# retinal-information-processing-lab/gaussian_processes

Measured on AMD Instinct MI355X. Metric: GP fits/sec (kernel+chol+solve+grad loglik) at N=8192 d=256, higher is better.
Workload: dtype f64; 1 GPU; N=8192 d=256 single cell f64, one M-step closure evaluation with 6 gradients (BASELINE configs[2], headline); N=8192, d=256, parallelism=independent units over 1 GPU(s), one process per GPU, no data-path collective

## Files before the change

gaussian_processes_amd/_lib.py:

```python
from __future__ import annotations

import ctypes
import os

from .build import lib_path

vp, i32, i64, f64 = ctypes.c_void_p, ctypes.c_int, ctypes.c_int64, ctypes.c_double
pd = ctypes.POINTER(ctypes.c_double)



class DevGemmArgs(ctypes.Structure):
    _fields_ = ([(n, vp) for n in ("A", "B", "C")] + [(n, i64) for n in ("lda", "ldb", "ldc", "sA", "sB", "sC")] +
                [("alpha", f64), ("beta", f64)] +
                [(n, vp) for n in ("sk_ws", "aux", "sumsq", "Ap", "Bp", "Cp", "auxp", "sumsqp")] +
                [(n, ctypes.c_int32) for n in ("M", "N", "K", "a_kmajor", "b_kmajor", "out_lower", "a_tri", "b_tri", "batch",
                                               "split_k", "tile", "walk", "epi", "nptr", "k_slabs")])


class DevGemmRoute(ctypes.Structure):
    _fields_ = [(n, ctypes.c_int32) for n in ("rc", "tile", "sk_first", "xcd", "stages", "half_occ", "edge", "epi",
                                              "sumsq_entries", "blocks", "pair", "slabs")]


_SIGS = {
    "gpfit_version": (i32, []),
    "gpfit_last_error": (ctypes.c_char_p, []),
    "gpfit_dgemm": (i32, [vp, i32, i32, i32, i32, i32, f64, vp, i64, vp, i64, f64, vp, i64, i32, i32, i32]),
    "gpfit_dgemm_ex": (i32, [vp, i32, i32, i32, i32, i32, f64, vp, i64, vp, i64, f64, vp, i64, i32, i32, i32, i32, i32]),
    "gpfit_ctx_create": (i32, [i32, i64, i64, i64, ctypes.POINTER(vp)]),
    "gpfit_ctx_destroy": (None, [vp]),
    "gpfit_check_limits": (i32, [pd, pd, pd]),
    "gpfit_localker_mask": (i32, [pd, i32, i32, vp, ctypes.POINTER(i64)]),
    "gpfit_localker": (i32, [vp, vp, pd, i32, i32, vp, i64, vp, vp]),
    "gpfit_acosker": (i32, [vp, vp, f64, vp, i64, i64, vp, i64, i64, i64, vp, i64, vp, vp, i64, vp]),
    "gpfit_acosker_pullback": (i32, [vp, vp, f64, vp, i64, i64, vp, i64, i64, i64, vp, i64, vp, i64, vp, vp, i64, pd]),
    "gpfit_acosker_diag": (i32, [vp, vp, f64, vp, i64, i64, i64, vp, i64, vp, vp, vp]),
    "gpfit_fit_eval": (i32, [vp, vp, pd, pd, pd, i32, i32, vp, i64, i64, vp, vp, vp, i64, f64, f64, i32, pd,
                             vp, vp, vp]),
    "gpfit_potrf": (i32, [vp, vp, vp, i64, i64, vp, i64, vp, i64, pd, ctypes.POINTER(i32)]),
    "gpfit_potrf_append": (i32, [vp, vp, vp, i64, vp, i64, i64, vp, pd, ctypes.POINTER(i32)]),
    "gpfit_estep": (i32, [vp, vp, vp, i64, i64, vp, vp, vp, f64, vp, vp, i64]),
    "gpfit_estep_projected": (i32, [vp, vp, vp, i64, vp, i64, vp, i64, i64, i64, vp, vp, vp, f64, vp, vp, i64, vp, vp,
                                    vp]),
    "gpfit_fparam_eval": (i32, [vp, vp, vp, vp, vp, i64, f64, i32, f64, vp, pd]),
    "gpfit_fparam_lbfgs": (i32, [vp, vp, vp, vp, vp, i64, f64, i32, f64, i32, i32, f64, f64, f64, vp, pd]),
    "gpfit_estep_chain": (i32, [vp, vp, vp, i64, vp, i64, vp, i64, i64, i64, vp, vp, vp, vp, vp, i64, vp, vp, f64, i32, f64,
                                i32, i32, i32, f64, f64, f64, pd]),
    "gpfit_estep_chain_full": (i32, [vp, vp, vp, i64, i64, vp, vp, vp, vp, vp, i64, vp, vp, f64, i32, f64, i32, i32, i32, f64,
                                     f64, f64, pd]),
    "gpfit_estep_chain_batch": (i32, [vp, i32, vp, vp, vp, vp, vp, vp, vp, i64, vp, vp, vp, vp, vp, vp, vp, vp, vp, pd, i32, pd,
                                      i32, i32, i32, f64, f64, f64, pd]),
    "gpfit_fparam_lbfgs_host": (i32, [vp, vp, vp, i64, f64, i32, f64, i32, i32, f64, f64, f64, vp, pd]),
    "gpfit_set_profile": (i32, [vp, i32]),
    "gpfit_get_profile": (i32, [vp, pd]),
    "gpfit_get_phases": (i32, [vp, pd]),
    "gpfit_last_enqueue_ms": (f64, [vp]),
    "gpfit_fit_eval_f32": (i32, [vp, vp, pd, pd, pd, i32, i32, vp, i64, i64, vp, vp, vp, i64, f64, f64, i32, pd,
                                 vp, vp, vp]),
    "gpfit_fit_eval_finish": (i32, [vp, pd]),
    "gpfit_fit_eval_batch": (i32, [vp, i32, vp, pd, pd, pd, i32, i32, vp, i64, i64, vp, vp, vp, i64, pd, pd, i32, pd,
                                   ctypes.POINTER(i32)]),
    "gpfit_fit_eval_batch_f32": (i32, [vp, i32, vp, pd, pd, pd, i32, i32, vp, i64, i64, vp, vp, vp, i64, pd, pd, i32, pd,
                                       ctypes.POINTER(i32)]),
    "gpfit_fit_eval_projected": (i32, [vp, vp, pd, pd, pd, i32, i32, vp, i64, i64, vp, vp, i64, i64, vp, vp, i64, f64, f64, pd]),
    "gpfit_fit_eval_sparse": (i32, [vp, vp, pd, pd, pd, i32, i32, vp, i64, i64, vp, i64, i64, vp, vp, i64, i64, vp, vp, i64,
                                    f64, f64, pd]),
    "gpfit_fit_eval_sparse_batch": (i32, [vp, i32, vp, pd, pd, pd, i32, i32, vp, i64, i64, vp, i64, i64, vp, vp, vp, vp, vp,
                                          vp, vp, pd, pd, pd, ctypes.POINTER(i32)]),
    "gpfit_grad_pullback": (i32, [vp, vp, pd, i32, i32, vp, i64, i64, vp, i64, vp, pd]),
    "gpfit_nd_utility": (i32, [vp, vp, vp, i64, vp, i32, vp]),
    "gpfit_probe_mfma_f64": (i32, [vp, vp, i32, i32]),
    "gpfit_probe_stream_copy": (i32, [vp, vp, vp, i64]),
    "gpfit_dev_gemm_route": (i32, [i32, ctypes.POINTER(DevGemmArgs), ctypes.POINTER(DevGemmArgs), ctypes.POINTER(DevGemmRoute)]),
    "gpfit_dev_gemm_plan": (i64, [i32, ctypes.POINTER(DevGemmArgs), i32, ctypes.POINTER(ctypes.c_int32), i64]),
    "gpfit_dev_gemm": (i32, [vp, i32, ctypes.POINTER(DevGemmArgs), ctypes.POINTER(DevGemmArgs)]),
    "gpfit_dev_ctx_copy": (i32, [vp, ctypes.c_char_p, i64, vp, i64, i32]),
    "gpfit_dev_ctx_fill": (i32, [vp, ctypes.c_char_p, i32]),
}

_lib = None


class GpfitError(RuntimeError):
    pass


def exported_symbols():
    return sorted(_SIGS)


def load():
    global _lib
    if _lib is not None:
        return _lib
    path = lib_path()
    if not os.path.exists(path):
        raise GpfitError(
            f"{path} not found: build it with `python -m gaussian_processes_amd.build` "
            "(there is no CPU fallback for the GP fit path)")
    lib = ctypes.CDLL(path)
    for name, (res, args) in _SIGS.items():
        fn = getattr(lib, name)
        fn.restype = res
        fn.argtypes = args
    _lib = lib
    return lib


def last_error() -> str:
    return load().gpfit_last_error().decode(errors="replace")


def check(rc: int, what: str):
    if rc < 0 and rc != -2:
        raise GpfitError(f"{what} failed (rc={rc}): {last_error()}")
    return rc


def darr(values):
    return (ctypes.c_double * len(values))(*[float(v) for v in values])
```

gaussian_processes_amd/csrc/api_dev.hip:

```cpp
#include "gemm_core.h"
#include "context.h"
#include "gpfit_mi355x.h"

#include <cstring>

namespace gpfit {
namespace {

template <typename R>
int fill(const gpfit_dev_gemm_args& d, GemmArgsT<R>& g) {
  g = GemmArgsT<R>{};
  g.A = (const R*)d.A; g.B = (const R*)d.B; g.C = (R*)d.C;
  g.lda = d.lda; g.ldb = d.ldb; g.ldc = d.ldc;
  g.M = d.M; g.N = d.N; g.K = d.K;
  g.alpha = d.alpha; g.beta = d.beta;
  g.a_kmajor = d.a_kmajor; g.b_kmajor = d.b_kmajor;
  g.out_lower = d.out_lower; g.a_tri = d.a_tri; g.b_tri = d.b_tri;
  g.batch = d.batch > 0 ? d.batch : 1;
  g.sA = d.sA; g.sB = d.sB; g.sC = d.sC;
  g.split_k = d.split_k > 0 ? d.split_k : 1;
  g.k_slabs = d.k_slabs > 0 ? d.k_slabs : 0;
  g.tile = d.tile;
  g.reverse = d.walk & 15;
  g.half_occ = (d.walk >> 4) & 1;
  g.sk_ws = d.sk_ws;
  g.epi = d.epi;
  g.aux = (R*)d.aux;
  g.sumsq = d.sumsq;
  g.nptr = d.nptr;
  if (d.nptr < 0 || d.nptr > GEMM_MAXB) return d.nptr < 0 ? -3 : 0;
  for (int b = 0; b < d.nptr; ++b) {
    if (!d.Ap || !d.Bp || !d.Cp) return -3;
    g.Ap[b] = (const R*)d.Ap[b];
    g.Bp[b] = (const R*)d.Bp[b];
    g.Cp[b] = (R*)d.Cp[b];
    g.auxp[b] = d.auxp ? (R*)d.auxp[b] : nullptr;
    g.sumsqp[b] = d.sumsqp ? d.sumsqp[b] : nullptr;
  }
  return 0;
}

template <typename R>
int route(const gpfit_dev_gemm_args& d, const gpfit_dev_gemm_args* d2, gpfit_dev_gemm_route_t& o) {
  std::memset(&o, 0, sizeof(o));
  o.sk_first = -1;
  GemmArgsT<R> a, b;
  if (fill(d, a) != 0 || (d2 && fill(*d2, b) != 0)) return -3;
  GemmRoute r = d2 ? gemm_pair_shape(a, b) : gemm_route(a);
  long blocks = d2 ? r.tiles : -1;
  if (r.rc == 0 && r.sched == GEMM_STREAMK) {
    SkHostPlan plan;
    if (streamk_plan_host(a, r.sk_first, plan) != 0) r.stay_data_parallel();
    else blocks = plan.blocks;
  }
  if (r.rc == 0 && r.sched == GEMM_XCD) {
    std::vector<int> table;
    if (xcd_plan_host(a, table) != 0) return -3;
    r.gx = (int)table.size();
  }
  o.rc = r.rc; o.tile = r.tile; o.sk_first = r.sk_first; o.xcd = r.sched == GEMM_XCD; o.stages = r.stages;
  o.half_occ = r.half; o.edge = r.edge; o.epi = r.epi; o.sumsq_entries = r.sumsq_entries; o.slabs = r.slabs;
  o.pair = d2 && r.rc == 0;
  o.blocks = (int)std::min<long>(blocks >= 0 ? blocks : (long)r.gx * r.gy * r.gz, 0x7fffffffL);
  return 0;
}

template <typename R>
int64_t plan(const gpfit_dev_gemm_args& d, int kind, int32_t* out, int64_t cap) {
  GemmArgsT<R> a;
  if (fill(d, a) != 0 || a.M <= 0 || a.N <= 0) return -3;
  const GemmRoute r = gemm_route(a);
  if (r.rc != 0) return -3;
  if (kind == 1) {
    if (r.sched != GEMM_XCD) return -1;
    std::vector<int> table;
    if (xcd_plan_host(a, table) != 0) return -1;
    const int64_t need = 1 + (int64_t)table.size();
    if (need > cap || !out) return need;
    out[0] = (int32_t)table.size();
    std::memcpy(out + 1, table.data(), table.size() * sizeof(int));
    return need;
  }
  if (kind == 3) {
    if (a.k_slabs <= 0) return -1;
    const SlabPlan sp = slab_plan(a.M, a.k_slabs);
    const int64_t need = 4 + 4 * (int64_t)sp.items;
    if (need > cap || !out) return need;
    out[0] = sp.items; out[1] = sp.live; out[2] = sp.ks * SLAB_TILE; out[3] = SLAB_TILE;
    for (int e = 0; e < sp.items; ++e) {
      int ti, z;
      slab_item(sp, e, ti, z);
      int32_t* w = out + 4 + 4 * e;
      w[0] = ti; w[1] = z;
      const KRange kr = gemm_tile_k_range(a.a_tri, a.b_tri, a.K, ti * SLAB_TILE, 0, SLAB_TILE);
      w[2] = std::max(kr.beg, z * sp.ks * SLAB_TILE);
      w[3] = std::min(kr.end, (z + 1) * sp.ks * SLAB_TILE);
    }
    return need;
  }
  if (kind != 2) return -3;
  if (r.sched != GEMM_STREAMK) return -1;
  const int first = r.sk_first;
  SkHostPlan p;
  if (streamk_plan_host(a, first, p) != 0) return -1;
  const int64_t nt = (int64_t)p.tiles.size(), nfix = (int64_t)p.fix_tile.size(), nslot = (int64_t)p.fix_slot.size();
  const int64_t need = 8 + 5 * nt + nfix + (nfix + 1) + nslot;
  if (need > cap || !out) return need;
  out[0] = first; out[1] = (int32_t)nt; out[2] = p.total; out[3] = p.blocks; out[4] = p.per_block;
  out[5] = (int32_t)nfix; out[6] = (int32_t)nslot;
  out[7] = (int32_t)(SK_WS_BYTES / ((size_t)TILE * TILE * sizeof(double)));
  int32_t* w = out + 8;
  for (const SkTile& t : p.tiles) { *w++ = t.row0; *w++ = t.col0; *w++ = t.kbeg; *w++ = t.ksteps; *w++ = t.prefix; }
  std::memcpy(w, p.fix_tile.data(), nfix * sizeof(int)); w += nfix;
  std::memcpy(w, p.fix_ptr.data(), (nfix + 1) * sizeof(int)); w += nfix + 1;
  std::memcpy(w, p.fix_slot.data(), nslot * sizeof(int));
  return need;
}

template <typename R>
int run(hipStream_t s, const gpfit_dev_gemm_args& d, const gpfit_dev_gemm_args* d2) {
  GemmArgsT<R> a, b;
  if (fill(d, a) != 0 || (d2 && fill(*d2, b) != 0)) {
    set_error("gpfit_dev_gemm: a pointer batch needs its pointer arrays");
    return -3;
  }
  return d2 ? launch_gemm_pair(a, b, gemm_pair_shape(a, b), s) : launch_gemm(a, s);
}

struct CtxBuf { void* p; int64_t bytes; };
CtxBuf ctx_buffer(gpfit_ctx* c, const char* name) {
  const int64_t np = c->np_cap, dp = c->dp_cap, nn = np * np * 8;
  const struct { const char* n; double* p; int64_t bytes; } tab[] = {
      {"Abuf", c->Abuf, nn}, {"Tbuf", c->Tbuf, nn}, {"Wbuf", c->Wbuf, nn}, {"Zbuf", c->Zbuf, nn}, {"Cos", c->Cos, nn},
      {"TmpV", c->TmpV, nn}, {"Xm", c->Xm, np * dp * 8}, {"Xt2", c->Xt2, np * dp * 8}, {"Ybuf", c->Ybuf, np * dp * 8},
      {"Mmat", c->Mmat, dp * dp * 8}, {"Cmat", c->Cmat, dp * dp * 8}, {"tvec", c->tvec, 2 * np * 8}, {"bv", c->bv, np * 8},
      {"q", c->q, np * 8}, {"wl", c->wl, np * 8}, {"q2", c->q2, np * 8}, {"dq1", c->dq1, np * 8}, {"dq2", c->dq2, np * 8}};
  for (const auto& t : tab)
    if (std::strcmp(t.n, name) == 0) return {t.p, t.bytes};
  return {nullptr, 0};
}

}
}

extern "C" {

int gpfit_dev_gemm_route(int is_f32, const gpfit_dev_gemm_args* args, const gpfit_dev_gemm_args* pair_args,
                         gpfit_dev_gemm_route_t* out) {
  if (!args || !out) return -3;
  return is_f32 ? gpfit::route<float>(*args, pair_args, *out) : gpfit::route<double>(*args, pair_args, *out);
}

int64_t gpfit_dev_gemm_plan(int is_f32, const gpfit_dev_gemm_args* args, int kind, int32_t* out, int64_t cap) {
  if (!args) return -3;
  return is_f32 ? gpfit::plan<float>(*args, kind, out, cap) : gpfit::plan<double>(*args, kind, out, cap);
}

int gpfit_dev_gemm(void* stream, int is_f32, const gpfit_dev_gemm_args* args, const gpfit_dev_gemm_args* pair_args) {
  if (!args) return -3;
  return is_f32 ? gpfit::run<float>((hipStream_t)stream, *args, pair_args)
                : gpfit::run<double>((hipStream_t)stream, *args, pair_args);
}

int gpfit_dev_ctx_copy(gpfit_ctx* ctx, const char* name, int64_t offset, void* dev, int64_t bytes, int to_ctx) {
  if (!ctx || !name || !dev || offset < 0 || bytes < 0 || ctx->pend.active) return -3;
  gpfit::DeviceGuard guard(ctx->device);
  const gpfit::CtxBuf b = gpfit::ctx_buffer(ctx, name);
  if (!b.p || offset + bytes > b.bytes) return -3;
  GP_HIP(hipDeviceSynchronize());
  char* w = (char*)b.p + offset;
  GP_HIP(hipMemcpy(to_ctx ? (void*)w : dev, to_ctx ? dev : (void*)w, (size_t)bytes, hipMemcpyDeviceToDevice));
  GP_HIP(hipDeviceSynchronize());
  return 0;
}

int gpfit_dev_ctx_fill(gpfit_ctx* ctx, const char* name, int byte) {
  if (!ctx || !name || ctx->pend.active) return -3;
  gpfit::DeviceGuard guard(ctx->device);
  const gpfit::CtxBuf b = gpfit::ctx_buffer(ctx, name);
  if (!b.p) return -3;
  GP_HIP(hipDeviceSynchronize());
  GP_HIP(hipMemset(b.p, byte, (size_t)b.bytes));
  GP_HIP(hipDeviceSynchronize());
  return 0;
}

}
```

gaussian_processes_amd/csrc/chol_leaf_reg.hip:

```cpp
#include "gemm_core.h"
#include "kernels.h"

#include <cstdlib>

namespace gpfit {

#ifdef GPFIT_LEAF_STAMPS
__device__ long long g_leaf_stamps[9 * 8];
__device__ long long g_leaf_wave_end[8 * 4];
#ifdef GPFIT_LEAF_STAMPS_MIN
#define LEAF_STAMP(kb, ph) do { if (((ph) == 3 || (kb) == 8) && (threadIdx.x & 63) == 0) g_leaf_stamps[(kb) * 8 + (ph)] = (long long)__builtin_readcyclecounter(); } while (0)
#else
#define LEAF_STAMP(kb, ph) do { if ((threadIdx.x & 63) == 0) g_leaf_stamps[(kb) * 8 + (ph)] = (long long)__builtin_readcyclecounter(); } while (0)
#endif
#define LEAF_WAVE_END(kb, w) do { if ((threadIdx.x & 63) == 0) g_leaf_wave_end[(kb) * 4 + (w)] = (long long)__builtin_readcyclecounter(); } while (0)
#else
#define LEAF_STAMP(kb, ph) do { } while (0)
#define LEAF_WAVE_END(kb, w) do { } while (0)
#endif

__device__ __forceinline__ void lds_barrier() { asm volatile("s_waitcnt lgkmcnt(0)\n\ts_barrier" ::: "memory"); }
__device__ __forceinline__ void lds_fence() { asm volatile("s_waitcnt lgkmcnt(0)" ::: "memory"); }

constexpr int RL = 128;
constexpr int RPS = 18;
constexpr int RL_THREADS = 320;
constexpr int RL_TILE_THREADS = 256;

__device__ __forceinline__ double rl_readlane(double v, int src_lane) {
  const int lo = __builtin_amdgcn_readlane(__double2loint(v), src_lane);
  const int hi = __builtin_amdgcn_readlane(__double2hiint(v), src_lane);
  return __hiloint2double(hi, lo);
}
__device__ __forceinline__ float rl_readlane(float v, int src_lane) {
  return __int_as_float(__builtin_amdgcn_readlane(__float_as_int(v), src_lane));
}
template <int J, typename R> __device__ __forceinline__ R rl_rowbcast(R x) {
  return __builtin_amdgcn_update_dpp(x, x, 0x150 + J, 0xf, 0xf, false);
}

__device__ __forceinline__ void rl_rsqrt_sqrt(double p, double& rinv, double& root) {
  double y = __builtin_amdgcn_rsq(p);
  const double hp = 0.5 * p;
  y = y * fma(-hp * y, y, 1.5);
#ifdef GPFIT_LEAF_TWO_NEWTON
  y = y * fma(-hp * y, y, 1.5);
#endif
  double d = p * y;
  d = fma(fma(-d, d, p), 0.5 * y, d);
  rinv = y;
  root = d;
}
__device__ __forceinline__ void rl_rsqrt_sqrt(float p, float& rinv, float& root) {
  float y = __builtin_amdgcn_rsqf(p);
  const float hp = 0.5f * p;
  y = y * fmaf(-hp * y, y, 1.5f);
  float d = p * y;
  d = fmaf(fmaf(-d, d, p), 0.5f * y, d);
  rinv = y;
  root = d;
}

template <int J> __device__ __forceinline__ double dpp_bcast_nop(double x) {
  double r;
  asm volatile("s_nop 1\n\tv_mov_b64_dpp %0, %1 row_newbcast:%2 row_mask:0xf bank_mask:0xf" : "=v"(r) : "v"(x), "n"(J));
  return r;
}
template <int J> __device__ __forceinline__ float dpp_bcast_nop(float x) {
  float r;
  asm volatile("s_nop 1\n\tv_mov_b32_dpp %0, %1 row_newbcast:%2 row_mask:0xf bank_mask:0xf" : "=v"(r) : "v"(x), "n"(J));
  return r;
}
template <int J, bool NOP> __device__ __forceinline__ void dpp_fmac(double& acc, double a, double b) {
  if constexpr (NOP)
    asm volatile("s_nop 1\n\tv_fmac_f64_dpp %0, %1, %2 row_newbcast:%3 row_mask:0xf bank_mask:0xf" : "+v"(acc) : "v"(a), "v"(b), "n"(J));
  else
    asm volatile("v_fmac_f64_dpp %0, %1, %2 row_newbcast:%3 row_mask:0xf bank_mask:0xf" : "+v"(acc) : "v"(a), "v"(b), "n"(J));
}
template <int J, bool NOP> __device__ __forceinline__ void dpp_fmac(float& acc, float a, float b) {
  if constexpr (NOP)
    asm volatile("s_nop 1\n\tv_fmac_f32_dpp %0, %1, %2 row_newbcast:%3 row_mask:0xf bank_mask:0xf" : "+v"(acc) : "v"(a), "v"(b), "n"(J));
  else
    asm volatile("v_fmac_f32_dpp %0, %1, %2 row_newbcast:%3 row_mask:0xf bank_mask:0xf" : "+v"(acc) : "v"(a), "v"(b), "n"(J));
}

template <int J, bool NOP> __device__ __forceinline__ void dpp_fmac_self(double& x, double b) {
  if constexpr (NOP)
    asm volatile("s_nop 1\n\tv_fmac_f64_dpp %0, %0, %1 row_newbcast:%2 row_mask:0xf bank_mask:0xf" : "+v"(x) : "v"(b), "n"(J));
  else
    asm volatile("v_fmac_f64_dpp %0, %0, %1 row_newbcast:%2 row_mask:0xf bank_mask:0xf" : "+v"(x) : "v"(b), "n"(J));
}
template <int J, bool NOP> __device__ __forceinline__ void dpp_fmac_self(float& x, float b) {
  if constexpr (NOP)
    asm volatile("s_nop 1\n\tv_fmac_f32_dpp %0, %0, %1 row_newbcast:%2 row_mask:0xf bank_mask:0xf" : "+v"(x) : "v"(b), "n"(J));
  else
    asm volatile("v_fmac_f32_dpp %0, %0, %1 row_newbcast:%2 row_mask:0xf bank_mask:0xf" : "+v"(x) : "v"(b), "n"(J));
}

template <typename R, int K, int J> __device__ __forceinline__ void static_for_cols(R (&v)[16], R vk, R nvk);
template <typename R, int K, int C> __device__ __forceinline__ void static_for_inv(R (&yh)[4], R m);

template <typename R, int K>
__device__ __forceinline__ void static_for_pivots(R (&v)[16], R (&yh)[4], R& myr, int& first_bad, int lane, int base) {
  if constexpr (K < 16) {
    R p = dpp_bcast_nop<K>(v[K]);
    const bool bad = !(p > (R)0);
    first_bad = (bad && first_bad == 0) ? (base + K + 1) : first_bad;
    p = bad ? (R)1 : p;
    R rinv, dkk;
    rl_rsqrt_sqrt(p, rinv, dkk);
    myr = (lane == K) ? rinv : myr;
    const R vk = (lane == K) ? dkk : v[K] * rinv;
    v[K] = vk;
    static_for_cols<R, K, K + 1>(v, vk, -vk);
    const R m = (lane > K) ? -vk * rinv : (R)0;
    static_for_inv<R, K, 0>(yh, m);
    static_for_pivots<R, K + 1>(v, yh, myr, first_bad, lane, base);
  }
}
template <typename R, int K, int J>
__device__ __forceinline__ void static_for_cols(R (&v)[16], R vk, R nvk) {
  if constexpr (J < 16) {
    dpp_fmac<J, J == K + 1>(v[J], vk, nvk);
    static_for_cols<R, K, J + 1>(v, vk, nvk);
  }
}
template <typename R, int K, int C>
__device__ __forceinline__ void static_for_inv(R (&yh)[4], R m) {
  if constexpr (4 * C <= K) {
    dpp_fmac_self<K, C == 0>(yh[C], m);
    static_for_inv<R, K, C + 1>(yh, m);
  }
}

constexpr int RL_SLOTS = 11;
__host__ __device__ constexpr int rl_col_a(int w) { return w == 0 ? 6 : w - 1; }
__host__ __device__ constexpr int rl_col_b(int w) { return w == 0 ? 7 : 6 - w; }
__host__ __device__ constexpr int rl_nslots(int w) { return (8 - rl_col_a(w)) + (8 - rl_col_b(w)); }
__host__ __device__ constexpr int rl_slot_i(int w, int t) { return t < 8 - rl_col_a(w) ? rl_col_a(w) + t : rl_col_b(w) + (t - (8 - rl_col_a(w))); }
__host__ __device__ constexpr int rl_slot_j(int w, int t) { return t < 8 - rl_col_a(w) ? rl_col_a(w) : rl_col_b(w); }

template <typename R, int W, int C, int T0>
__device__ __forceinline__ void leaf_update_column(typename Real<R>::acc_t (&acc)[RL_SLOTS], const R* __restrict__ P,
                                                   const R (&dneg)[4], const typename Real<R>::acc_t& dvt, R* __restrict__ RawN,
                                                   R* __restrict__ Dg0, R* __restrict__ Dg1, int kb, const int (&kr)[4], int fr) {
  using Acc = typename Real<R>::acc_t;
  constexpr int NR = 8 - C;
  const int nx = kb + 1;
  R fa[2][4];
  auto row_frag = [&](int i, R (&f)[4]) {
#pragma unroll
    for (int r = 0; r < 4; ++r) f[r] = P[(16 * i + fr) * RPS + kr[r]];
  };
  if (C > kb) {
    R nfb[4];
#pragma unroll
    for (int r = 0; r < 4; ++r) nfb[r] = -P[(16 * C + fr) * RPS + kr[r]];
    row_frag(C, fa[0]);
#pragma unroll
    for (int t = 0; t < NR; ++t) {
      const int i = C + t;
      Acc& a = acc[T0 + t];
      if (t + 1 < NR) row_frag(i + 1, fa[(t + 1) & 1]);
      const R (&f)[4] = fa[t & 1];
      if (!(t == 0 && C == nx)) {
#pragma unroll
        for (int r = 0; r < 4; ++r) a = Real<R>::mfma(f[r], nfb[r], a);
      }
      if (C == nx && t > 0) {
#pragma unroll
        for (int r = 0; r < 4; ++r) RawN[(16 * i + kr[r]) * RPS + fr] = a[r];
      } else if (C == nx + 1 && t == 0) {
        R* Dg = (C & 1) ? Dg1 : Dg0;
#pragma unroll
        for (int r = 0; r < 4; ++r) Dg[kr[r] * RPS + fr] = a[r];
      }
      __builtin_amdgcn_sched_barrier(0);
    }
  } else {
    Acc xrow = acc_zero<R>();
#pragma unroll
    for (int t = 0; t < NR; ++t) {
      if (C + t == kb) {
        if (C == kb) {
          xrow = dvt;
        } else {
#pragma unroll
          for (int r = 0; r < 4; ++r) xrow = Real<R>::mfma(dneg[r], acc[T0 + t][r], xrow);
        }
        acc[T0 + t] = xrow;
      }
    }
    row_frag(C, fa[0]);
#pragma unroll
    for (int t = 0; t < NR; ++t) {
      const int i = C + t;
      Acc& a = acc[T0 + t];
      if (t + 1 < NR) row_frag(i + 1, fa[(t + 1) & 1]);
      const R (&f)[4] = fa[t & 1];
      if (i > kb) {
        if (C == kb) a = acc_zero<R>();
#pragma unroll
        for (int r = 0; r < 4; ++r) a = Real<R>::mfma(f[r], xrow[r], a);
      }
      __builtin_amdgcn_sched_barrier(0);
    }
  }
}

template <typename R, int W>
__device__ __forceinline__ void leaf_update_pass(typename Real<R>::acc_t (&acc)[RL_SLOTS], const R* __restrict__ P,
                                                 const R* __restrict__ Dv, R* __restrict__ RawN, R* __restrict__ Dg0,
                                                 R* __restrict__ Dg1, int kb, const int (&kr)[4], int fr) {
  using Acc = typename Real<R>::acc_t;
  constexpr int CA = rl_col_a(W), CB = rl_col_b(W);
  R dneg[4];
  Acc dvt;
#pragma unroll
  for (int r = 0; r < 4; ++r) {
    dneg[r] = -Dv[fr * RPS + kr[r]];
    dvt[r] = Dv[kr[r] * RPS + fr];
  }
  leaf_update_column<R, W, CA, 0>(acc, P, dneg, dvt, RawN, Dg0, Dg1, kb, kr, fr);
  leaf_update_column<R, W, CB, 8 - CA>(acc, P, dneg, dvt, RawN, Dg0, Dg1, kb, kr, fr);
}

template <typename R, int W>
__device__ __forceinline__ void leaf_load_tiles(typename Real<R>::acc_t (&acc)[RL_SLOTS], const R* __restrict__ A, int64_t lda,
                                                R* __restrict__ Raw0, R* __restrict__ Dg0, R* __restrict__ Dg1,
                                                const int (&kr)[4], int fr) {
#pragma unroll
  for (int t = 0; t < RL_SLOTS; ++t) {
    if (t >= rl_nslots(W)) { acc[t] = acc_zero<R>(); continue; }
    const int i = rl_slot_i(W, t), j = rl_slot_j(W, t);
#pragma unroll
    for (int r = 0; r < 4; ++r) acc[t][r] = A[(int64_t)(16 * i + kr[r]) * lda + 16 * j + fr];
    if (j == 0 && i > 0) {
#pragma unroll
      for (int r = 0; r < 4; ++r) Raw0[(16 * i + kr[r]) * RPS + fr] = acc[t][r];
    }
    if (i == j && j <= 1) {
      R* Dg = j ? Dg1 : Dg0;
#pragma unroll
      for (int r = 0; r < 4; ++r) Dg[kr[r] * RPS + fr] = acc[t][r];
    }
  }
}
template <typename R, int W>
__device__ __forceinline__ void leaf_store_inverse(const typename Real<R>::acc_t (&acc)[RL_SLOTS], R* __restrict__ Linv,
                                                   int64_t ldi, const int (&kr)[4], int fr) {
#pragma unroll
  for (int t = 0; t < rl_nslots(W); ++t) {
    const int i = rl_slot_i(W, t), j = rl_slot_j(W, t);
#pragma unroll
    for (int r = 0; r < 4; ++r) Linv[(int64_t)(16 * i + kr[r]) * ldi + 16 * j + fr] = acc[t][r];
  }
}

template <typename R>
__global__ __launch_bounds__(RL_THREADS, 2) void chol_leaf_reg_kernel(LeafBatchT<R> bt) {
  const R* __restrict__ A = bt.A[blockIdx.x];
  R* __restrict__ L = bt.L[blockIdx.x];
  R* __restrict__ Linv = bt.Li[blockIdx.x];
  int* __restrict__ info = bt.info[blockIdx.x];
  const int64_t lda = bt.lda, ldl = bt.ldl, ldi = bt.ldi;
  const int info_base = bt.info_base;
  using Acc = typename Real<R>::acc_t;
  using V = typename Real<R>::vec_t;
  constexpr int EPC = Real<R>::EPC;
  __shared__ __attribute__((aligned(16))) R Rawb[1][RL * RPS];
  __shared__ __attribute__((aligned(16))) R Lpb[1][RL * RPS];
  __shared__ __attribute__((aligned(16))) R Dbuf[2][16 * RPS];
  __shared__ __attribute__((aligned(16))) R Dgb[2][16 * RPS];
  __shared__ __attribute__((aligned(16))) R Sx[16 * RPS];
  __shared__ unsigned b2_arrivals;
  const int tid = threadIdx.x, lane = tid & 63;
  const int wave = __builtin_amdgcn_readfirstlane(tid >> 6);
  const int fr = lane & 15;
  int kr[4];
#pragma unroll
  for (int r = 0; r < 4; ++r) kr[r] = Real<R>::crow(lane, r);

  if (tid == 0) b2_arrivals = 0u;
  auto b2_arrive = [&]() {
    asm volatile("s_waitcnt lgkmcnt(0)" ::: "memory");
    if (lane == 0) __hip_atomic_fetch_add(&b2_arrivals, 1u, __ATOMIC_RELAXED, __HIP_MEMORY_SCOPE_WORKGROUP);
  };
  auto b2_wait = [&](unsigned target) {
    while (__hip_atomic_load(&b2_arrivals, __ATOMIC_RELAXED, __HIP_MEMORY_SCOPE_WORKGROUP) < target) { }
    asm volatile("" ::: "memory");
  };
  if (wave == 4) {
    __builtin_amdgcn_s_setprio(3);
    LEAF_STAMP(8, 0);
    auto pivot_block = [&](int nx, int lane_o) {
      const int li = lane_o & 15, lg = lane_o >> 4;
      R v[16], yh[4];
      {
        const R* row = Sx + li * RPS;
#pragma unroll
        for (int q = 0; q < 16 / EPC; ++q) {
          const V w = *reinterpret_cast<const V*>(row + EPC * q);
#pragma unroll
          for (int e = 0; e < EPC; ++e) v[EPC * q + e] = w[e];
        }
      }
#pragma unroll
      for (int c = 0; c < 4; ++c) yh[c] = (4 * c + lg == li) ? (R)1 : (R)0;
      int first_bad = 0;
      R myr = (R)0;
      LEAF_STAMP(nx, 1);
      static_for_pivots<R, 0>(v, yh, myr, first_bad, li, 16 * nx);
      LEAF_STAMP(nx, 2);
      if (lane == 0 && first_bad != 0) atomicCAS(info, 0, info_base + first_bad);
      {
        R* drow = Dbuf[nx & 1] + li * RPS + lg;
#pragma unroll
        for (int c = 0; c < 4; ++c) drow[4 * c] = yh[c] * myr;
      }
      if (lane < 16) {
        R* grow = L + (int64_t)(16 * nx + lane) * ldl + 16 * nx;
#pragma unroll
        for (int q = 0; q < 16 / EPC; ++q) {
          V lv;
#pragma unroll
          for (int e = 0; e < EPC; ++e) {
            const int j = EPC * q + e;
            lv[e] = (j <= lane) ? v[j] : (R)0;
          }
          *reinterpret_cast<V*>(grow + EPC * q) = lv;
        }
      }
      LEAF_STAMP(nx, 3);
    };
    {
      int lane_o = lane;
      asm volatile("" : "+v"(lane_o));
      if (lane < 16) {
        const R* arow = A + (int64_t)lane * lda;
        R* srow = Sx + lane * RPS;
#pragma unroll
        for (int q = 0; q < 16 / EPC; ++q) *reinterpret_cast<V*>(srow + EPC * q) = *reinterpret_cast<const V*>(arow + EPC * q);
      }
      lds_fence();
      pivot_block(0, lane_o);
    }
    lds_barrier();
#pragma unroll 1
    for (int kb = 0; kb < 8; ++kb) {
      int lane_o = lane;
      asm volatile("" : "+v"(lane_o));
      const int nx = kb + 1;
      const R* const Raw = Rawb[0];
      const R* const Dv = Dbuf[kb & 1];
      lds_barrier();
      LEAF_STAMP(kb, 4);
      if (nx < 8) {
        Acc lt = acc_zero<R>();
#pragma unroll
        for (int r = 0; r < 4; ++r) lt = Real<R>::mfma(Dv[fr * RPS + kr[r]], Raw[(16 * nx + fr) * RPS + kr[r]], lt);
        Acc sd;
#pragma unroll
        for (int r = 0; r < 4; ++r) sd[r] = Dgb[nx & 1][kr[r] * RPS + fr];
        b2_arrive();
#pragma unroll
        for (int r = 0; r < 4; ++r) sd = Real<R>::mfma(-lt[r], lt[r], sd);
#pragma unroll
        for (int r = 0; r < 4; ++r) Sx[kr[r] * RPS + fr] = sd[r];
        lds_fence();
      } else {
        b2_arrive();
      }
      LEAF_STAMP(kb, 5);
      if (nx < 8) {
        LEAF_STAMP(nx, 0);
        pivot_block(nx, lane_o);
      }
    }
    return;
  }

  Acc acc[RL_SLOTS];
  switch (wave) {
    case 0: leaf_load_tiles<R, 0>(acc, A, lda, Rawb[0], Dgb[0], Dgb[1], kr, fr); break;
    case 1: leaf_load_tiles<R, 1>(acc, A, lda, Rawb[0], Dgb[0], Dgb[1], kr, fr); break;
    case 2: leaf_load_tiles<R, 2>(acc, A, lda, Rawb[0], Dgb[0], Dgb[1], kr, fr); break;
    default: leaf_load_tiles<R, 3>(acc, A, lda, Rawb[0], Dgb[0], Dgb[1], kr, fr); break;
  }
  lds_barrier();

#pragma unroll 1
  for (int kb = 0; kb < 8; ++kb) {
    int lane_o = lane;
    asm volatile("" : "+v"(lane_o));
    const int fr = lane_o & 15;
    int kr[4];
#pragma unroll
    for (int r = 0; r < 4; ++r) kr[r] = Real<R>::crow(lane_o, r);
    const R* const Raw = Rawb[0];
    R* const P = Lpb[0];
    const R* const Dv = Dbuf[kb & 1];
    R* const RawN = Rawb[0];

    lds_barrier();
    {
      Acc s0 = acc_zero<R>(), s1 = acc_zero<R>();
      const int i0 = kb + 1 + wave, i1 = kb + 5 + wave;
      const int c0 = i0 < 8 ? i0 : 7, c1 = i1 < 8 ? i1 : 7;
      {
        R a0[4], a1[4], dd[4];
#pragma unroll
        for (int r = 0; r < 4; ++r) {
          a0[r] = Raw[(16 * c0 + fr) * RPS + kr[r]];
          a1[r] = Raw[(16 * c1 + fr) * RPS + kr[r]];
          dd[r] = Dv[fr * RPS + kr[r]];
        }
#pragma unroll
        for (int r = 0; r < 4; ++r) {
          s0 = Real<R>::mfma(a0[r], dd[r], s0);
          s1 = Real<R>::mfma(a1[r], dd[r], s1);
        }
      }
      if (i0 < 8) {
#pragma unroll
        for (int r = 0; r < 4; ++r) {
          P[(16 * i0 + kr[r]) * RPS + fr] = s0[r];
          L[(int64_t)(16 * i0 + kr[r]) * ldl + 16 * kb + fr] = s0[r];
        }
      }
      if (i1 < 8) {
#pragma unroll
        for (int r = 0; r < 4; ++r) {
          P[(16 * i1 + kr[r]) * RPS + fr] = s1[r];
          L[(int64_t)(16 * i1 + kr[r]) * ldl + 16 * kb + fr] = s1[r];
        }
      }
    }
    b2_arrive();
    b2_wait(5u * (unsigned)(kb + 1));
    switch (wave) {
      case 0: leaf_update_pass<R, 0>(acc, P, Dv, RawN, Dgb[0], Dgb[1], kb, kr, fr); break;
      case 1: leaf_update_pass<R, 1>(acc, P, Dv, RawN, Dgb[0], Dgb[1], kb, kr, fr); break;
      case 2: leaf_update_pass<R, 2>(acc, P, Dv, RawN, Dgb[0], Dgb[1], kb, kr, fr); break;
      default: leaf_update_pass<R, 3>(acc, P, Dv, RawN, Dgb[0], Dgb[1], kb, kr, fr); break;
    }
    if (wave == 0) {
      const int row = 16 * kb + (lane_o >> 2), cq = 4 * (lane_o & 3);
      V zero2;
#pragma unroll
      for (int e = 0; e < EPC; ++e) zero2[e] = (R)0;
      for (int tj = kb + 1; tj < 8; ++tj) {
        R* lrow = L + (int64_t)row * ldl + 16 * tj + cq;
        R* irow = Linv + (int64_t)row * ldi + 16 * tj + cq;
#pragma unroll
        for (int q = 0; q < 4 / EPC; ++q) {
          *reinterpret_cast<V*>(lrow + EPC * q) = zero2;
          *reinterpret_cast<V*>(irow + EPC * q) = zero2;
        }
      }
      LEAF_STAMP(kb, 6);
    }
    LEAF_WAVE_END(kb, wave);
  }

  switch (wave) {
    case 0: leaf_store_inverse<R, 0>(acc, Linv, ldi, kr, fr); break;
    case 1: leaf_store_inverse<R, 1>(acc, Linv, ldi, kr, fr); break;
    case 2: leaf_store_inverse<R, 2>(acc, Linv, ldi, kr, fr); break;
    default: leaf_store_inverse<R, 3>(acc, Linv, ldi, kr, fr); break;
  }
  LEAF_STAMP(8, 1);
}

template <typename R>
int launch_chol_leaf_batch(const LeafBatchT<R>& bt, hipStream_t s) {
  if (bt.n <= 0 || bt.n > GEMM_MAXB) {
    set_error("launch_chol_leaf_batch: 1 .. GEMM_MAXB blocks per launch");
    return -3;
  }
  hipLaunchKernelGGL(chol_leaf_reg_kernel<R>, dim3(bt.n), dim3(RL_THREADS), 0, s, bt);
  GP_HIP(hipGetLastError());
  return 0;
}

template int launch_chol_leaf_batch<double>(const LeafBatchT<double>&, hipStream_t);
template int launch_chol_leaf_batch<float>(const LeafBatchT<float>&, hipStream_t);

}
```

gaussian_processes_amd/csrc/context.h:

```cpp
#pragma once
#include "kernels.h"
#include <vector>

struct gpfit_ctx {
  int device = 0;
  int np_cap = 0, dp_cap = 0, dfull_cap = 0;
  hipStream_t aux = nullptr;
  hipEvent_t ev_fork = nullptr, ev_join = nullptr;

  double *Kbuf = nullptr, *Cos = nullptr, *Lbuf = nullptr, *Libuf = nullptr, *Vbuf = nullptr, *LVbuf = nullptr,
         *LiVbuf = nullptr, *Tbuf = nullptr, *Zbuf = nullptr, *Wbuf = nullptr, *Abuf = nullptr, *Tmp = nullptr,
         *TmpV = nullptr;
  double *Xt = nullptr, *Xm = nullptr, *XCt = nullptr, *Cmat = nullptr, *Ybuf = nullptr, *Mpart = nullptr,
         *Mmat = nullptr, *Xt2 = nullptr, *XCt2 = nullptr, *XDt = nullptr, *XDt2 = nullptr, *dCpad = nullptr;
  double *Kvec = nullptr, *q = nullptr, *lam_m = nullptr, *lam_var = nullptr, *fvec = nullptr, *wl = nullptr,
         *yv = nullptr, *bv = nullptr, *tvec = nullptr , *mpad = nullptr, *rpad = nullptr,
         *q2 = nullptr, *dq1 = nullptr, *dq2 = nullptr, *hvec = nullptr;
  double *upart = nullptr, *vpart = nullptr, *sumA_part = nullptr, *frob_part = nullptr, *trmv_part = nullptr;
  double* rect_part = nullptr;
  void* sk_ws[2] = {nullptr, nullptr};
  hipStream_t side = nullptr;
  std::vector<hipEvent_t> side_ev;
  int side_ev_next = 0;
  double* scal = nullptr;
  double* scal_host = nullptr;
  int* pix = nullptr;
  int* pix_host = nullptr;
  int* info = nullptr;
  int* info_host = nullptr;
  gpfit::ChainBlock* chain = nullptr;
  double* chain_host = nullptr;
  std::vector<void*> allocs;
  int split_k_M = 32;

  int profile = 0;
  struct ProfRec { hipEvent_t a, b; double flops; int kind; };
  std::vector<ProfRec> prof;
  std::vector<hipEvent_t> ev_pool;
  double prof_out[16] = {0};
  hipEvent_t phase_ev[8] = {nullptr, nullptr, nullptr, nullptr, nullptr, nullptr, nullptr, nullptr};
  bool phase_valid = false;
  double last_enqueue_ms = 0.0;
  struct Pending { bool active = false; hipStream_t stream = nullptr; double A = 0, lambda0 = 0, sigma0 = 0;
                   int n = 0, np = 0, d = 0, want_grad = 0, elem_bytes = 8; hipEvent_t done = nullptr;
                   bool use_done = false; } pend;

  int cur_n = 0, cur_np = 0, cur_d = 0, cur_dp = 0;
  bool lv_valid = false;
  bool lv32_valid = false;
  int lv_n = 0;
  int lv_bytes = 0;
};

namespace gpfit {

struct Lane { hipStream_t s; void* sk_ws; };
inline Lane main_lane(const gpfit_ctx* c, hipStream_t s) { return {s, c->sk_ws[0]}; }
inline Lane side_lane(const gpfit_ctx* c) { return {c->side, c->sk_ws[1]}; }

enum ScalSlot {
  S_RLAM = 0, S_SUMR = 1, S_SUMF = 2,
  S_LOGDET_K = 3,
  S_TRACE = 5,
  S_MKM = 6,
  S_ADJ = 7, S_ADJ_WL = 8, S_ADJ_SUMA = 9,
  S_METRIC = 10,
  S_D_AMP = 10, S_D_BETA = 11, S_D_RHO = 12, S_D_EPSX = 13, S_D_EPSY = 14,
  S_RECT = 20, S_RECT_U1 = 21, S_RECT_U2 = 22,
  S_FPARAM = 32,
  S_LOGDET_V = 40,
  S_APPEND = 48, S_APPEND_LAMBDA = 49,
  S_LBFGS = 52,
};
enum InfoWord {
  INFO_K = 0, INFO_V = 1,
  INFO_MOMENTS = 2,
  INFO_METRIC = 3,
};
enum Walk { W_TRSM, W_TMP, W_MERGE, W_T, W_Q, W_RBASE, W_H, W_COUNT };
enum OutSlot {
  OUT_LOSS = 0, OUT_LOGLIK = 1, OUT_KL = 2, OUT_GRAD = 3 , OUT_LOGDET_K = 9, OUT_LOGDET_V = 10, OUT_TRACE = 11,
  OUT_MKM = 12, OUT_D = 13, OUT_INFO_K = 14, OUT_INFO_V = 15, OUT_COUNT = 16,
};

struct DeviceGuard {
  int prev = -1;
  bool switched = false;
  explicit DeviceGuard(int device) {
    if (hipGetDevice(&prev) == hipSuccess && prev != device) switched = (hipSetDevice(device) == hipSuccess);
  }
  ~DeviceGuard() {
    if (switched) (void)hipSetDevice(prev);
  }
};
#define GP_CTX_ENTER(c, name)                                                                        \
  if ((c)->pend.active) {                                                                            \
    gpfit::set_error(name ": an asynchronous evaluation is pending on this context (collect it with " \
                          "gpfit_fit_eval_finish first)");                                           \
    return -3;                                                                                       \
  }                                                                                                  \
  gpfit::DeviceGuard _device_guard((c)->device)

void prof_begin(gpfit_ctx* c);
void prof_end(gpfit_ctx* c);
struct ProfScope {
  hipStream_t s; double flops; int kind; hipEvent_t a = nullptr;
  ProfScope(hipStream_t s, double flops, int kind);
  ~ProfScope();
};
template <typename R> double gemm_flops(const GemmArgsT<R>& g, int tile);

template <typename R>
struct CholBatchT {
  int nb = 0;
  R* A[GEMM_MAXB];
  R* L[GEMM_MAXB];
  R* Li[GEMM_MAXB];
  R* Tmp[GEMM_MAXB];
  int* info[GEMM_MAXB];
  int64_t ld = 0;
  gpfit_ctx* ctx = nullptr;
  int side_min = 0;
};
template <typename R>
int potrf_lockstep(const CholBatchT<R>& B, int r0, int n, uint32_t need, Lane lane, uint32_t halves = 0);

}
```

gaussian_processes_amd/csrc/fit.hip:

```cpp
#include "product.h"
#include "gemm_core.h"
#include "gpfit_mi355x.h"

#include <algorithm>
#include <chrono>
#include <cmath>
#include <cstdlib>
#include <cstring>
#include <limits>

namespace gpfit {

static thread_local gpfit_ctx* g_prof = nullptr;

static int walk(Walk which) {
  static int w[W_COUNT] = {3, 2, 1, 9, 9, 2, 2};
  static bool init = false;
  if (!init) {
    init = true;
    if (const char* e = getenv("GPFIT_WALKS")) {
      int v[W_COUNT];
      if (sscanf(e, "%d,%d,%d,%d,%d,%d,%d", &v[0], &v[1], &v[2], &v[3], &v[4], &v[5], &v[6]) == 7)
        for (int i = 0; i < W_COUNT; ++i) w[i] = v[i];
    }
  }
  return w[which];
}

static hipEvent_t prof_event(gpfit_ctx* c) {
  hipEvent_t e;
  if (!c->ev_pool.empty()) {
    e = c->ev_pool.back();
    c->ev_pool.pop_back();
    return e;
  }
  (void)hipEventCreate(&e);
  return e;
}

void prof_begin(gpfit_ctx* c) {
  if (c->profile == 1) {
    g_prof = c;
    c->prof.clear();
  }
}

void prof_end(gpfit_ctx* c) {
  if (g_prof != c) return;
  g_prof = nullptr;
  (void)hipDeviceSynchronize();
  double ms[4] = {0, 0, 0, 0}, fl[4] = {0, 0, 0, 0}, cnt[4] = {0, 0, 0, 0};
  double big_ms = 0, big_fl = 0;
  for (auto& r : c->prof) {
    float t = 0.f;
    (void)hipEventElapsedTime(&t, r.a, r.b);
    if (r.kind == 0 && r.flops > big_fl) { big_fl = r.flops; big_ms = t; }
    ms[r.kind] += t;
    fl[r.kind] += r.flops;
    cnt[r.kind] += 1;
    c->ev_pool.push_back(r.a);
    c->ev_pool.push_back(r.b);
  }
  c->prof.clear();
  c->prof_out[0] = ms[0]; c->prof_out[1] = fl[0]; c->prof_out[2] = cnt[0];
  c->prof_out[3] = ms[1]; c->prof_out[4] = cnt[1];
  c->prof_out[5] = ms[2]; c->prof_out[6] = fl[2]; c->prof_out[7] = cnt[2];
  c->prof_out[8] = ms[3]; c->prof_out[9] = fl[3]; c->prof_out[10] = cnt[3];
  c->prof_out[11] = big_ms; c->prof_out[12] = big_fl;
}

ProfScope::ProfScope(hipStream_t s_, double flops_, int kind_) : s(s_), flops(flops_), kind(kind_) {
  if (g_prof) {
    a = prof_event(g_prof);
    (void)hipEventRecord(a, s);
  }
}
ProfScope::~ProfScope() {
  if (g_prof && a) {
    hipEvent_t b = prof_event(g_prof);
    (void)hipEventRecord(b, s);
    g_prof->prof.push_back({a, b, flops, kind});
  }
}

template <typename R>
double gemm_flops(const GemmArgsT<R>& g, int T) {
  const int tm = (g.M + T - 1) / T, tn = (g.N + T - 1) / T, r = TILE / T;
  double steps = 0;
  for (int ti = 0; ti < tm; ++ti)
    for (int tj = 0; tj < tn; ++tj) {
      if (g.out_lower && tj / r > ti / r) continue;
      const KRange kr = gemm_tile_k_range(g.a_tri, g.b_tri, g.K, ti * T, tj * T, T);
      if (kr.end > kr.beg) steps += (kr.end - kr.beg);
    }
  return 2.0 * T * T * steps * (g.nptr > 0 ? g.nptr : (g.batch > 0 ? g.batch : 1));
}

static int g_eval_count = 0;
static int gemm_log_eval() {
  static const int v = getenv("GPFIT_GEMM_LOG") ? atoi(getenv("GPFIT_GEMM_LOG")) : -1;
  return v;
}
static bool gemm_logging() { return gemm_log_eval() >= 0 && g_eval_count == gemm_log_eval(); }
template <typename R>
static void gemm_log_tail(const char* tag, const GemmArgsT<R>& g, const char* end) {
  fprintf(stderr, "%s alpha %g beta %g lda %lld ldb %lld ldc %lld walk %d split %d slabs %d%s", tag, g.alpha, g.beta, (long long)g.lda,
          (long long)g.ldb, (long long)g.ldc, g.reverse, g.split_k, g.k_slabs, end);
}

template <typename R>
int run_gemm(hipStream_t s, const GemmArgsT<R>& g, const GemmRoute& r) {
  if (gemm_logging()) {
    fprintf(stderr, "[gpfit gemm] M %d N %d K %d atri %d btri %d lower %d nb %d tile %d ak %d bk %d epi %d flops %.6e", g.M, g.N, g.K,
            g.a_tri, g.b_tri, g.out_lower, g.nptr > 0 ? g.nptr : 1, r.tile, g.a_kmajor, g.b_kmajor, g.epi, gemm_flops(g, r.tile));
    gemm_log_tail("", g, "\n");
  }
  ProfScope ps(s, g_prof ? gemm_flops(g, r.tile) : 0.0, (g_prof && r.tile != TILE) ? 3 : 0);
  return launch_gemm(g, r, s);
}
template int run_gemm<double>(hipStream_t, const GemmArgsT<double>&, const GemmRoute&);
template int run_gemm<float>(hipStream_t, const GemmArgsT<float>&, const GemmRoute&);

static int splitk_for(int M, int N, int K) {
  const long tiles = (long)((M + TILE - 1) / TILE) * ((N + TILE - 1) / TILE);
  if (tiles >= 384) return 1;
  long sp = (768 + tiles - 1) / tiles;
  sp = std::min<long>(sp, std::max(1, K / 256));
  return (int)std::max<long>(1, sp);
}
template <typename R>
static int gemm_splitk(Lane lane, Dims d, double alpha, const Operand<R>& a, const Operand<R>& b, R* C, int64_t ldc, R* partial,
                       int64_t partial_elems) {
  static const bool off = getenv("GPFIT_NO_SPLITK") != nullptr;
  const int64_t slab = (int64_t)d.M * ldc;
  const int splits = (int)std::min<int64_t>(splitk_for(d.M, d.N, d.K),
                                            partial_elems / std::max<int64_t>(1, slab));
  if (splits <= 1 || off || partial == nullptr) return product(lane, d, alpha, a, b, into(mat(C, ldc)));
  GemmArgsT<R> g = product_args(lane, d, alpha, a, b, into(mat(partial, ldc)));
  g.split_k = splits;
  g.sC = slab;
  g.tile = TILE;
  GP_TRY(run_gemm(lane.s, g));
  return launch_reduce_slices(partial, slab, splits, C, slab, lane.s);
}

template <typename R>
static int gemm_splitk_list(Lane lane, Dims d, double alpha, const Operand<R>& a, const Operand<R>& b, const Mat<R>& C,
                            R* const* partial, const int64_t* partial_elems) {
  static const bool off = getenv("GPFIT_NO_SPLITK") != nullptr;
  const int cnt = C.cnt;
  const int64_t slab = (int64_t)d.M * C.ld;
  bool any = false;
  for (int i = 0; i < cnt && !off; ++i)
    any = any || (partial[i] && std::min<int64_t>(splitk_for(d.M, d.N, d.K), partial_elems[i] / std::max<int64_t>(1, slab)) > 1);
  if (!any) return product(lane, d, alpha, a, b, into(C));
  for (int i = 0; i < cnt; ++i) {
    Operand<R> ai = a, bi = b;
    ai.m.cnt = bi.m.cnt = 1;
    ai.m.p[0] = a.m.p[i]; bi.m.p[0] = b.m.p[i];
    GP_TRY(gemm_splitk(lane, d, alpha, ai, bi, C.p[i], C.ld, partial[i], partial_elems[i]));
  }
  return 0;
}

static int fused_epilogues() {
  static const int v = getenv("GPFIT_FUSED_EPI") ? atoi(getenv("GPFIT_FUSED_EPI")) : 7;
  return v;
}

template <typename R>
int product(Lane lane, Dims d, double alpha, const Operand<R>& a, const Operand<R>& b, const Output<R>& c, int walk, Epilogue<R>* e) {
  const int cnt = c.m.cnt, epi = e ? e->which : 0;
  if (e) { e->carried = false; e->sumsq_entries = 0; }
  if (cnt <= 0) return 0;
  if (cnt > GEMM_MAXB) {
    set_error("product: more problems than a pointer batch holds");
    return -3;
  }
  GemmArgsT<R> g = product_args(lane, d, alpha, a, b, c, walk);
  static const bool no_batch = getenv("GPFIT_NO_BATCH") != nullptr;
  if (cnt == 1 || gemm_pick_tile(g) == TILE || no_batch) {
    auto problem = [&](int i, bool fused) {
      g.A = a.m.p[i]; g.B = b.m.p[i]; g.C = c.m.p[i];
      g.epi = fused ? epi : 0; g.aux = fused ? e->aux[i] : nullptr; g.sumsq = fused ? e->sumsq[i] : nullptr;
    };
    GemmRoute routes[GEMM_MAXB];
    bool fused = epi != 0;
    for (int i = 0; i < cnt && fused; ++i) {
      problem(i, true);
      routes[i] = gemm_route(g);
      fused = routes[i].epi != 0;
    }
    for (int i = 0; i < cnt; ++i) {
      problem(i, fused);
      GP_TRY(fused ? run_gemm(lane.s, g, routes[i]) : run_gemm(lane.s, g));
    }
    if (e) e->carried = fused;
    if (fused) e->sumsq_entries = routes[0].sumsq_entries;
    return 0;
  }
  g = batch_args(lane, d, alpha, a, b, c, walk, e);
  GemmRoute r = gemm_route(g);
  if (epi && r.epi == 0) {
    g.epi = 0;
    r = gemm_route(g);
  }
  if (e) { e->carried = g.epi != 0; e->sumsq_entries = r.sumsq_entries; }
  return run_gemm(lane.s, g, r);
}
template int product<double>(Lane, Dims, double, const Operand<double>&, const Operand<double>&, const Output<double>&, int,
                             Epilogue<double>*);
template int product<float>(Lane, Dims, double, const Operand<float>&, const Operand<float>&, const Output<float>&, int,
                            Epilogue<float>*);

template <typename R>
int potrf_lockstep(const CholBatchT<R>& B, int r0, int n, uint32_t need, Lane lane, uint32_t halves) {
  const int64_t ld = B.ld;
  const hipStream_t s = lane.s;
  const uint32_t all = (B.nb >= 32) ? 0xffffffffu : ((1u << B.nb) - 1u);
  auto off = [&](int r, int c) { return (int64_t)r * ld + c; };
  auto blk = [&](uint32_t mask, R* const* X, int r, int c) {
    Mat<R> m{};
    m.ld = ld;
    for (int b = 0; b < B.nb; ++b)
      if (mask & (1u << b)) m.p[m.cnt++] = X[b] + off(r, c);
    return m;
  };
  if (n == TILE) {
    ProfScope ps(s, 0.0, 1);
    LeafBatchT<R> bt{};
    bt.n = B.nb;
    for (int b = 0; b < B.nb; ++b) {
      bt.A[b] = B.A[b] + off(r0, r0); bt.L[b] = B.L[b] + off(r0, r0); bt.Li[b] = B.Li[b] + off(r0, r0);
      bt.info[b] = B.info[b];
    }
    bt.lda = bt.ldl = bt.ldi = ld;
    bt.info_base = r0;
    return launch_chol_leaf_batch(bt, s);
  }
  const int k = n / TILE;
  const int n1 = ((k + 1) / 2) * TILE, n2 = n - n1;
  const int r1 = r0 + n1;
  GP_TRY(potrf_lockstep<R>(B, r0, n1, all, lane));
  GP_TRY(product(lane, {n2, n1, n1}, 1.0, plain(blk(all, B.A, r1, r0)), trans(tril(blk(all, B.Li, r0, r0))),
                 into(blk(all, B.L, r1, r0)), walk(W_TRSM)));
  const Operand<R> L21 = plain(blk(all, B.L, r1, r0)), L21t = trans(blk(all, B.L, r1, r0));
  const Output<R> A22 = into_lower(blk(all, B.A, r1, r1), 1.0);
  const Operand<R> L21n = plain(blk(need, B.L, r1, r0)), Li11 = plain(tril(blk(need, B.Li, r0, r0)));
  const Output<R> tmp = into(blk(need, B.Tmp, r1, r0));
  const Dims syrk{n2, n2, n1}, merge1{n2, n1, n1};
  hipEvent_t joined = nullptr;
  if (need && B.ctx && B.side_min > 0 && n >= B.side_min && B.ctx->side) {
    gpfit_ctx* c = B.ctx;
    auto next_event = [&]() {
      if (c->side_ev_next == (int)c->side_ev.size()) {
        hipEvent_t e = nullptr;
        (void)hipEventCreateWithFlags(&e, hipEventDisableTiming);
        c->side_ev.push_back(e);
      }
      return c->side_ev[c->side_ev_next++];
    };
    hipEvent_t fork = next_event();
    joined = next_event();
    GP_HIP(hipEventRecord(fork, s));
    GP_HIP(hipStreamWaitEvent(c->side, fork, 0));
    GP_TRY(product(side_lane(c), merge1, 1.0, L21n, Li11, tmp, walk(W_TMP)));
    GP_HIP(hipEventRecord(joined, c->side));
  }
  bool merged = false;
  if (need && !joined) {
    static const bool no_batch = getenv("GPFIT_NO_BATCH") != nullptr;
    const GemmArgsT<R> g2 = batch_args(lane, syrk, -1.0, L21, L21t, A22);
    const GemmArgsT<R> g3 = batch_args(lane, merge1, 1.0, L21n, Li11, tmp, walk(W_TMP));
    const GemmRoute pr = no_batch ? GemmRoute{} : gemm_pair_shape(g2, g3);
    if (!no_batch && pr.rc == 0) {
      if (gemm_logging()) {
        fprintf(stderr, "[gpfit gemm] pair: M %d N %d K %d lower 1 nb %d + M %d N %d K %d btri 1 nb %d tile %d flops %.6e", g2.M, g2.N,
                g2.K, g2.nptr, g3.M, g3.N, g3.K, g3.nptr, pr.tile, gemm_flops(g2, pr.tile) + gemm_flops(g3, pr.tile));
        gemm_log_tail(" a:", g2, "");
        gemm_log_tail(" b:", g3, "\n");
      }
      ProfScope ps(s, g_prof ? gemm_flops(g2, pr.tile) + gemm_flops(g3, pr.tile) : 0.0, 3);
      GP_TRY(launch_gemm_pair(g2, g3, pr, s));
      merged = true;
    }
  }
  if (!merged) GP_TRY(product(lane, syrk, -1.0, L21, L21t, A22));
  GP_TRY(potrf_lockstep<R>(B, r1, n2, need | halves, lane));
  if (need) {
    if (joined) GP_HIP(hipStreamWaitEvent(s, joined, 0));
    else if (!merged) GP_TRY(product(lane, merge1, 1.0, L21n, Li11, tmp, walk(W_TMP)));
    GP_TRY(product(lane, {n2, n1, n2}, -1.0, plain(tril(blk(need, B.Li, r1, r1))), plain(blk(need, B.Tmp, r1, r0)),
                   into(blk(need, B.Li, r1, r0)), walk(W_MERGE)));
  }
  return 0;
}

template int potrf_lockstep<double>(const CholBatchT<double>&, int, int, uint32_t, Lane, uint32_t);
template int potrf_lockstep<float>(const CholBatchT<float>&, int, int, uint32_t, Lane, uint32_t);

template <typename R>
struct TwoSidedBufs { R* Q; const R* Li; R *W, *Z, *H; const R* L; int64_t ld; int min_split; };
template <typename R, typename P>
static Mat<P> ts_blk(int cnt, const TwoSidedBufs<R>* b, const int* r0, P* TwoSidedBufs<R>::*X, int dr, int dc) {
  return mats(cnt, b[0].ld, [&](int i) { const int o = r0 ? r0[i] : 0; return b[i].*X + (int64_t)(o + dr) * b[i].ld + o + dc; });
}
template <typename R>
static int dual_update_list(Lane lane, Dims d, double alpha, const Operand<R>& a, const Operand<R>& b, const Mat<R>& H,
                            const Mat<R>& Z, int wk) {
  const int cnt = H.cnt;
  const int64_t ld = H.ld;
  Epilogue<R> e{4};
  for (int i = 0; i < cnt; ++i) e.aux[i] = Z.p[i];
  bool fused = false;
  if (fused_epilogues() & 4) {
    GemmArgsT<R> g = product_args(lane, d, alpha, a, b, into(H), wk);
    g.epi = 4; g.aux = Z.p[0];
    static const bool no_batch = getenv("GPFIT_NO_BATCH") != nullptr;
    if (cnt > 1 && gemm_pick_tile(g) != TILE && !no_batch) { g.nptr = cnt; g.batch = cnt; }
    fused = gemm_route(g).epi != 0;
  }
  if (fused) {
    GP_TRY(product(lane, d, alpha, a, b, into(H), wk, &e));
    if (!e.carried) {
      set_error("two_sided: the dual-update epilogue was announced but not carried");
      return -100;
    }
    return 0;
  }
  for (int i = 0; i < cnt; ++i)
    GP_HIP(hipMemcpy2DAsync(H.p[i], (size_t)ld * sizeof(R), Z.p[i], (size_t)ld * sizeof(R), (size_t)d.N * sizeof(R), (size_t)d.M,
                            hipMemcpyDeviceToDevice, lane.s));
  GP_TRY(product(lane, d, alpha, a, b, into(H, 1.0), wk));
  for (int i = 0; i < cnt; ++i) GP_TRY(launch_axpby_block<R>(Z.p[i], ld, H.p[i], ld, d.M, d.N, 1.0, 1.0, lane.s));
  return 0;
}

template <typename R>
static int two_sided_list(Lane lane, int cnt, const TwoSidedBufs<R>* b, const int* r0, int n) {
  if (cnt <= 0) return 0;
  using TS = TwoSidedBufs<R>;
  auto blk = [&](auto X, int dr, int dc) { return ts_blk(cnt, b, r0, X, dr, dc); };
  const int k = n / TILE;
  if (n < b[0].min_split || k < 2) {
    static const int wbase_walk = getenv("GPFIT_WBASE_WALK") ? atoi(getenv("GPFIT_WBASE_WALK")) : 0;
    GP_TRY(product(lane, {n, n, n}, 1.0, trans(blk(&TS::Q, 0, 0)), plain(tril(blk(&TS::Li, 0, 0))), into(blk(&TS::Z, 0, 0)),
                   walk(W_RBASE)));
    return product(lane, {n, n, n}, 0.5, trans(tril(blk(&TS::Li, 0, 0))), plain(blk(&TS::Z, 0, 0)),
                   into_lower(blk(&TS::W, 0, 0)), wbase_walk);
  }
  const int n1 = ((k + 1) / 2) * TILE, n2 = n - n1;
  auto diagonal_blocks = [&]() -> int {
    TwoSidedBufs<R> bb[GEMM_MAXB];
    int rr[GEMM_MAXB];
    if (n1 == n2 && 2 * cnt <= GEMM_MAXB) {
      for (int i = 0; i < cnt; ++i) {
        bb[2 * i] = b[i]; rr[2 * i] = r0[i];
        bb[2 * i + 1] = b[i]; rr[2 * i + 1] = r0[i] + n1;
      }
      return two_sided_list<R>(lane, 2 * cnt, bb, rr, n1);
    }
    for (int i = 0; i < cnt; ++i) rr[i] = r0[i] + n1;
    GP_TRY(two_sided_list<R>(lane, cnt, b, r0, n1));
    return two_sided_list<R>(lane, cnt, b, rr, n2);
  };
  GP_TRY(product(lane, {n2, n1, n2}, 0.5, trans(blk(&TS::Q, n1, n1)), plain(blk(&TS::Li, n1, 0)), into(blk(&TS::Z, n1, 0))));
  GP_TRY(dual_update_list(lane, {n2, n1, n1}, 1.0, plain(blk(&TS::Q, n1, 0)), plain(tril(blk(&TS::Li, 0, 0))), blk(&TS::H, n1, 0),
                          blk(&TS::Z, n1, 0), walk(W_H)));
  static const int w21_walk = getenv("GPFIT_W21_WALK") ? atoi(getenv("GPFIT_W21_WALK")) : 0;
  GP_TRY(product(lane, {n2, n1, n2}, 0.5, trans(tril(blk(&TS::Li, n1, n1))), plain(blk(&TS::Z, n1, 0)),
                 into(blk(&TS::W, n1, 0)), w21_walk));
  GP_TRY(diagonal_blocks());
  GP_TRY(product(lane, {n1, n1, n2}, 0.5, trans(blk(&TS::Li, n1, 0)), plain(blk(&TS::H, n1, 0)), into_lower(blk(&TS::W, 0, 0), 1.0)));
  return product(lane, {n1, n1, n2}, 0.5, trans(blk(&TS::H, n1, 0)), plain(blk(&TS::Li, n1, 0)), into_lower(blk(&TS::W, 0, 0), 1.0));
}

constexpr int TOP_BLOCKS_MIN = 2048, TOP_BLOCKS_MIN_F32 = 5120;
static bool top_in_blocks(int np, size_t elem_bytes) { return np >= (elem_bytes == 4 ? TOP_BLOCKS_MIN_F32 : TOP_BLOCKS_MIN); }

template <typename R>
static int two_sided_top(Lane lane, int cnt, const TwoSidedBufs<R>* b, int n) {
  if (cnt <= 0) return 0;
  using TS = TwoSidedBufs<R>;
  const hipStream_t s = lane.s;
  const int64_t ld = b[0].ld;
  auto blk = [&](auto X, int r, int c) { return ts_blk(cnt, b, (const int*)nullptr, X, r, c); };
  int rr[GEMM_MAXB];
  const int k = n / TILE;
  const int n1 = ((k + 1) / 2) * TILE, n2 = n - n1;
  for (int i = 0; i < cnt; ++i) rr[i] = n1;
  GP_TRY(two_sided_list<R>(lane, cnt, b, rr, n2));
  for (int i = 0; i < cnt; ++i) GP_TRY(launch_symmetrize(b[i].W + (int64_t)n1 * ld + n1, ld, n2, s));
  static const int w21_walk = getenv("GPFIT_W21_WALK") ? atoi(getenv("GPFIT_W21_WALK")) : 0;
  GP_TRY(product(lane, {n2, n1, n2}, 0.5, trans(tril(blk(&TS::Li, n1, n1))), plain(blk(&TS::Q, n1, 0)),
                 into(blk(&TS::Z, n1, 0)), w21_walk));
  GP_TRY(dual_update_list(lane, {n2, n1, n2}, -1.0, plain(blk(&TS::W, n1, n1)), plain(blk(&TS::L, n1, 0)), blk(&TS::H, n1, 0),
                          blk(&TS::Z, n1, 0), 0));
  GP_TRY(product(lane, {n2, n1, n1}, 1.0, plain(blk(&TS::H, n1, 0)), plain(tril(blk(&TS::Li, 0, 0))), into(blk(&TS::W, n1, 0)),
                 walk(W_H)));
  GP_TRY(product(lane, {n1, n1, n2}, -1.0, trans(blk(&TS::L, n1, 0)), plain(blk(&TS::Z, n1, 0)), into_lower(blk(&TS::Q, 0, 0), 1.0)));
  GP_TRY(product(lane, {n1, n1, n2}, -1.0, trans(blk(&TS::Z, n1, 0)), plain(blk(&TS::L, n1, 0)), into_lower(blk(&TS::Q, 0, 0), 1.0)));
  for (int i = 0; i < cnt; ++i) GP_TRY(launch_symmetrize(b[i].Q, ld, n1, s));
  for (int i = 0; i < cnt; ++i) rr[i] = 0;
  return two_sided_list<R>(lane, cnt, b, rr, n1);
}

static double lin_pm1_host(int i, int n) {
  if (n <= 1) return -1.0;
  const double step = 2.0 / (double)(n - 1);
  return (i < n / 2) ? std::fma(step, (double)i, -1.0) : std::fma(-step, (double)(n - 1 - i), 1.0);
}

static int compute_mask(const double* theta, int n_rows, int n_cols, uint8_t* mask, int* pix) {
  const double eb = std::exp(theta[3]);
  int d = 0;
  for (int p = 0; p < n_rows * n_cols; ++p) {
    const double x = lin_pm1_host(p % n_cols, n_cols), y = lin_pm1_host(p / n_cols, n_rows);
    const double dx = x - theta[1], dy = y - theta[2];
    const double alpha = std::exp(-eb * (dx * dx + dy * dy));
    const bool keep = alpha >= 0.001;
    if (mask) mask[p] = keep ? 1 : 0;
    if (keep) {
      if (pix) pix[d] = p;
      ++d;
    }
  }
  return d;
}

static Theta make_theta(const double* t) {
  Theta th;
  th.sigma0 = t[0]; th.eps0x = t[1]; th.eps0y = t[2]; th.logbeta = t[3]; th.logrho = t[4]; th.amp = t[5];
  th.eb = std::exp(t[3]);
  th.er = std::exp(t[4]);
  return th;
}

static int check_limits(const double* theta, const double* lower, const double* upper) {
  static const char* names[6] = {"sigma_0", "eps_0x", "eps_0y", "-2log2beta", "-log2rho2", "Amp"};
  for (int i = 0; i < 6; ++i) {
    if (!(lower[i] <= theta[i] && theta[i] <= upper[i])) {
      char buf[256];
      snprintf(buf, sizeof buf, "%s = %.4f is not within the limits of %g and %g", names[i], theta[i], lower[i],
               upper[i]);
      set_error(buf);
      return -2;
    }
  }
  return 0;
}

static int ensure_side_stream(gpfit_ctx* c) {
  if (c->side) return 0;
  int least = 0, greatest = 0;
  GP_HIP(hipDeviceGetStreamPriorityRange(&least, &greatest));
  GP_HIP(hipStreamCreateWithPriority(&c->side, hipStreamNonBlocking, least));
  return 0;
}

template <typename T>
static int dev_alloc(gpfit_ctx* c, T** p, size_t count) {
  void* q = nullptr;
  GP_HIP(hipMalloc(&q, count * sizeof(T)));
  c->allocs.push_back(q);
  *p = (T*)q;
  return 0;
}

template <typename R>
static R* ws_as(double* b) { return reinterpret_cast<R*>(b); }

static void fill_out_of_box(double* out) {
  const double inf = std::numeric_limits<double>::infinity();
  out[OUT_LOSS] = inf;
  out[OUT_LOGLIK] = out[OUT_KL] = std::numeric_limits<double>::quiet_NaN();
  for (int i = 0; i < 6; ++i) out[OUT_GRAD + i] = inf;
}

struct Admitted { int d, dp; Theta th; };
static int admit(gpfit_ctx* c, const char* name, const char* whose, const double* theta, const double* lower,
                 const double* upper, int n_rows, int n_cols, int np, double* out, Admitted* a) {
  if (lower && upper && check_limits(theta, lower, upper) != 0) {
    fill_out_of_box(out);
    return -2;
  }
  if (np > c->np_cap || n_rows * n_cols > c->dfull_cap) {
    set_error(std::string(name) + ": problem larger than " + whose + " capacity");
    return -3;
  }
  a->d = compute_mask(theta, n_rows, n_cols, nullptr, c->pix_host);
  a->dp = (int)round_up(a->d, 32);
  if (a->d <= 0 || a->dp > c->dp_cap) {
    set_error(std::string(name) + ": masked pixel count is zero or exceeds " + whose + " capacity");
    return -3;
  }
  a->th = make_theta(theta);
  return 0;
}

template <typename R>
static int build_metric(gpfit_ctx* c, hipStream_t s, const Theta& th, int d, int dp, int n_rows, int n_cols) {
  return launch_localker<R>(th, c->pix, d, dp, n_rows, n_cols, ws_as<R>(c->Cmat), dp, nullptr, s);
}
template <typename R>
static int kernel_side(gpfit_ctx* c, Lane lane, const R* X, int64_t ldx, int n, int np, int d, int dp, double s0sq,
                       R* Xt, R* XCt, R* Xm, R* Kvec, R* q) {
  const int64_t ld = np;
  const hipStream_t s = lane.s;
  GP_TRY(launch_gather(X, ldx, n, c->pix, d, dp, np, Xt, ld, Xm, dp, s));
  GP_TRY(product(lane, {dp, np, dp}, 1.0, trans(mat(ws_as<R>(c->Cmat), dp)), plain(mat(Xt, ld)), into(mat(XCt, ld))));
  return launch_qvec(Xt, XCt, ld, dp, n, np, s0sq, Kvec, q, s);
}
template <typename R>
static int gram_square(hipStream_t s, const R* XCt, const R* Xt, const R* q, R* Kout, R* Cos, int n, int np, int dp,
                       double s0sq, int mirror) {
  GramArgsT<R> g{};
  g.XCt = XCt; g.Xt = Xt; g.q1 = q; g.q2 = q; g.Kout = Kout; g.Cos = Cos;
  g.ld1 = np; g.ld2 = np; g.ldk = np; g.np1 = np; g.np2 = np; g.nv1 = n; g.nv2 = n; g.Kd = dp;
  g.s0sq = s0sq; g.lower = 1; g.pad_identity = 1;
  g.mirror = mirror;
  ProfScope ps(s, (double)np * (np + TILE) * dp, 2);
  return launch_gram(g, s);
}
template <typename R>
static int build_kernel(gpfit_ctx* c, Lane lane, const Theta& th, int d, int dp, int n_rows, int n_cols, const R* X,
                        int64_t ldx, int n, int np, int mirror) {
  const double s0sq = th.sigma0 * th.sigma0;
  const hipStream_t s = lane.s;
  GP_TRY(build_metric<R>(c, s, th, d, dp, n_rows, n_cols));
  GP_TRY(kernel_side<R>(c, lane, X, ldx, n, np, d, dp, s0sq, ws_as<R>(c->Xt), ws_as<R>(c->XCt), ws_as<R>(c->Xm),
                        ws_as<R>(c->Kvec), ws_as<R>(c->q)));
  return gram_square<R>(s, ws_as<R>(c->XCt), ws_as<R>(c->Xt), ws_as<R>(c->q), ws_as<R>(c->Kbuf), ws_as<R>(c->Cos), n, np,
                        dp, s0sq, mirror);
}

template <typename R>
static int solve_mean(gpfit_ctx* c, int np, bool blocks, hipStream_t s) {
  const int64_t ld = np;
  R *m = ws_as<R>(c->mpad), *y = ws_as<R>(c->yv), *b = ws_as<R>(c->bv);
  if (!blocks) {
    GP_TRY(launch_trmv_lower(ws_as<R>(c->Libuf), ld, np, m, y, s));
    GP_TRY(launch_dot(y, y, np, c->scal + S_MKM, s));
    return launch_trmv_lower_t(ws_as<R>(c->Libuf), ld, np, y, b, c->trmv_part, s);
  }
  const int kt = np / TILE, n1 = ((kt + 1) / 2) * TILE, n2 = np - n1;
  const R *A = ws_as<R>(c->Libuf), *C = A + (int64_t)n1 * ld + n1, *L21 = ws_as<R>(c->Lbuf) + (int64_t)n1 * ld;
  GP_TRY(launch_trmv_lower(A, ld, n1, m, y, s));
  GP_TRY(launch_gemv_sub(L21, ld, n2, n1, y, m + n1, b + n1, s));
  GP_TRY(launch_trmv_lower(C, ld, n2, b + n1, y + n1, s));
  GP_TRY(launch_dot(y, y, np, c->scal + S_MKM, s));
  GP_TRY(launch_trmv_lower_t(C, ld, n2, y + n1, b + n1, c->trmv_part, s));
  GP_TRY(launch_gemv_t_sub(L21, ld, n2, n1, b + n1, y, b, c->trmv_part, s));
  return launch_trmv_lower_t(A, ld, n1, b, b, c->trmv_part, s);
}

template <typename R>
static int adjoint_pass(gpfit_ctx* c, hipStream_t s, const R* W, const R* Cos, const R* bv, const R* q, const R* wl, int n,
                        int np, R* A, R* tvec) {
  GP_TRY(launch_adjoint(W, Cos, (int64_t)np, bv, q, n, np, A, c->upart, c->vpart, c->sumA_part, s));
  const int t64 = np / 64;
  return launch_adjoint_reduce(c->upart, c->vpart, c->sumA_part, t64, t64 * (t64 + 1) / 2, q, wl, n, np, tvec, c->rpad,
                               c->scal + S_ADJ, s);
}
template <typename R>
static int xty(gpfit_ctx* c, hipStream_t s, const R* Xa, const R* Yb, int np, int dp, R* out, bool prof, bool sym = false) {
  GemmArgsT<R> g = product_args(Lane{s, nullptr}, {dp, dp, np}, 1.0, trans(mat(Xa, dp)), plain(mat(Yb, dp)),
                                into(mat(ws_as<R>(c->Mpart), dp)));
  g.split_k = c->split_k_M; g.sC = (int64_t)dp * dp;
  const GemmRoute r = gemm_route(g);
  if (prof) {
    ProfScope ps(s, g_prof ? gemm_flops(g, r.tile) : 0.0, (g_prof && r.tile != TILE) ? 3 : 0);
    GP_TRY(launch_gemm(g, r, s));
  } else {
    GP_TRY(launch_gemm(g, r, s));
  }
  if (sym) return launch_reduce_slices_sym(ws_as<R>(c->Mpart), (int64_t)dp * dp, c->split_k_M, out, dp, s);
  return launch_reduce_slices(ws_as<R>(c->Mpart), (int64_t)dp * dp, c->split_k_M, out, (int64_t)dp * dp, s);
}
static int pullback_slabs(int np, int dp) {
  const int nt = np / SLAB_TILE;
  return std::max(1, std::min(nt >= 32 ? 4 : (nt >= 8 ? 2 : 1), np / dp));
}
template <typename R>
static int lambda_t_x_list(Lane lane, const Operand<R>& a, const Operand<R>& b, const Mat<R>& Y, const Mat<R>& scratch, int np, int dp) {
  const int cnt = Y.cnt;
  if (cnt <= 0 || cnt > GEMM_MAXB) return cnt == 0 ? 0 : -3;
  const int slabs = pullback_slabs(np, dp);
  const SlabPlan sp = slab_plan(np, slabs);
  const bool direct = sp.live == 1;
  const Output<R> c = into(direct ? Y : scratch);
  GemmArgsT<R> g = cnt > 1 ? batch_args(lane, {np, dp, np}, 1.0, a, b, c) : product_args(lane, {np, dp, np}, 1.0, a, b, c);
  g.k_slabs = slabs;
  g.sC = (int64_t)np * dp;
  GP_TRY(run_gemm(lane.s, g));
  if (direct) return 0;
  for (int i = 0; i < cnt; ++i)
    GP_TRY(launch_reduce_slabs(scratch.p[i], (int64_t)np * dp, sp.live, sp.ks * SLAB_TILE, Y.p[i], np, dp, lane.s));
  return 0;
}
static int pullback_to_metric(gpfit_ctx* c, Lane lane, const double* W, const double* Cos, const double* q, int n,
                              int np, int dp, double* A, const double* Xm, double* scratch) {
  const hipStream_t s = lane.s;
// ... 1096 lines not shown
```

gaussian_processes_amd/csrc/gemm.hip:

```cpp
#include "gemm_core.h"

#include <algorithm>
#include <cstdlib>
#include <mutex>
#include <set>
#include <utility>

namespace gpfit {

template <typename R, bool A_KMAJOR, bool B_KMAJOR, bool EDGE, int T, int NS>
__device__ __forceinline__ bool gemm_tile_compute(const GemmArgsT<R>& p, int tiles_n, int ntiles, R* smem,
                                                  typename Real<R>::acc_t (&acc)[T / 32][T / 32], int& ti, int& tj,
                                                  int& row0, int& col0, R*& C) {
  constexpr int KT = Real<R>::KT;

  int slab = 0, slab_tiles = 0;
  const bool slabbed = (T == SLAB_TILE) && p.k_slabs > 0;
  if (slabbed) {
    const SlabPlan sp = slab_plan(p.M, p.k_slabs);
    slab_item(sp, (int)blockIdx.x / tiles_n, ti, slab);
    tj = (int)blockIdx.x % tiles_n;
    slab_tiles = sp.ks;
  } else if (p.sched != nullptr) {
    const int e = p.sched[blockIdx.x];
    if (e < 0) return false;
    ti = e >> 16;
    tj = e & 0xffff;
  } else {
    gemm_walk_tile((int)blockIdx.x, p.reverse, p.out_lower != 0, TILE / T, tiles_n, ntiles, ti, tj);
  }
  row0 = ti * T;
  col0 = tj * T;
  const int b = blockIdx.y, z = blockIdx.z;
  const R* A;
  const R* B;
  if (p.nptr > 0) {
    A = p.Ap[b];
    B = p.Bp[b];
    C = p.Cp[b];
  } else {
    A = p.A + (int64_t)b * p.sA;
    B = p.B + (int64_t)b * p.sB;
    C = p.C + (int64_t)b * p.sC;
  }

  const KRange kr = gemm_tile_k_range(p.a_tri, p.b_tri, p.K, row0, col0, T);
  int kbeg = kr.beg, kend = kr.end;
  if (slabbed) {
    kbeg = max(kbeg, slab * slab_tiles * T);
    kend = min(kend, (slab + 1) * slab_tiles * T);
    C += (int64_t)slab * p.sC;
  } else if (p.split_k > 1) {
    const int steps = max(0, kend - kbeg) / KT;
    const int per = (steps + p.split_k - 1) / p.split_k;
    const int s0 = min(steps, z * per), s1 = min(steps, (z + 1) * per);
    kend = kbeg + s1 * KT;
    kbeg = kbeg + s0 * KT;
    C += (int64_t)z * p.sC;
  }

#pragma unroll
  for (int i = 0; i < T / 32; ++i)
#pragma unroll
    for (int j = 0; j < T / 32; ++j) acc[i][j] = acc_zero<R>();

  gemm_mainloop<R, A_KMAJOR, B_KMAJOR, EDGE, T, 0, NS>(A, p.lda, B, p.ldb, p.M, p.N, row0, col0, kbeg, kend, smem, acc,
                                                       (p.reverse & 4) != 0);
  return true;
}

template <typename R, bool A_KMAJOR, bool B_KMAJOR, bool EDGE, int T, int NS, int EPI = 0>
__device__ __forceinline__ void gemm_tile_body(const GemmArgsT<R>& p, int tiles_n, int ntiles, R* smem) {
  typename Real<R>::acc_t acc[T / 32][T / 32];
  int ti, tj, row0, col0;
  R* C;
  if (!gemm_tile_compute<R, A_KMAJOR, B_KMAJOR, EDGE, T, NS>(p, tiles_n, ntiles, smem, acc, ti, tj, row0, col0, C)) return;

  const R alpha = (R)p.alpha, beta = (p.split_k > 1 || (T == SLAB_TILE && p.k_slabs > 0)) ? (R)0 : (R)p.beta;
  const int64_t ldc = p.ldc;
  const int M = p.M, N = p.N;
  if constexpr (EPI != 0) {
    constexpr int epi = EPI;
    R* __restrict__ D = p.nptr > 0 ? p.auxp[blockIdx.y] : p.aux;
    double* __restrict__ sumsq = p.nptr > 0 ? p.sumsqp[blockIdx.y] : p.sumsq;
    double ss = 0.0;
    for_each_acc<R, T>(acc, row0, col0, [&](int row, int col, R v) {
      if (EDGE && !(row < M && col < N)) return;
      R o = alpha * v;
      R* c = C + (int64_t)row * ldc + col;
      if (epi & 4) {
        R* dd = D + (int64_t)row * ldc + col;
        const R d0 = *dd;
        o += d0;
        *dd = o + d0;
      } else if (beta != (R)0) {
        o += beta * (*c);
      }
      if (epi & 1) {
        if (row >= col) *c = o;
        if (row > col) C[(int64_t)col * ldc + row] = o;
      } else {
        *c = o;
      }
      if (epi & 2) ss += (double)o * (double)o;
    });
    if (epi & 2) {
#pragma unroll
      for (int o = 32; o > 0; o >>= 1) ss += __shfl_down(ss, o);
      double* red = reinterpret_cast<double*>(smem);
      __syncthreads();
      if ((threadIdx.x & 63) == 0) red[threadIdx.x >> 6] = ss;
      __syncthreads();
      if (threadIdx.x == 0)
        sumsq[p.out_lower ? (int64_t)ti * (ti + 1) / 2 + tj : (int64_t)ti * tiles_n + tj] = (red[0] + red[1]) + (red[2] + red[3]);
    }
    return;
  }
  if (beta == (R)0) {
    for_each_acc<R, T>(acc, row0, col0, [&](int row, int col, R v) {
      if (!EDGE || (row < M && col < N)) C[(int64_t)row * ldc + col] = alpha * v;
    });
  } else {
    for_each_acc<R, T>(acc, row0, col0, [&](int row, int col, R v) {
      if (!EDGE || (row < M && col < N)) {
        R* c = C + (int64_t)row * ldc + col;
        *c = alpha * v + beta * (*c);
      }
    });
  }
}

template <typename R, bool A_KMAJOR, bool B_KMAJOR, bool EDGE, int T, int NS = 2>
__global__ __launch_bounds__(GEMM_THREADS, (T == 128 || NS > 2 ? 2 : 4)) void gemm_mfma_kernel(GemmArgsT<R> p,
                                                                                               int tiles_n,
                                                                                               int ntiles) {
  __shared__ __attribute__((aligned(16))) R smem[2 * NS * Real<R>::KT * T];
  gemm_tile_body<R, A_KMAJOR, B_KMAJOR, EDGE, T, NS>(p, tiles_n, ntiles, smem);
}

#ifdef GPFIT_CLOCK_STAMPS
__device__ long long g_gemm_clock[2][4096][2];
#endif

template <typename R, bool A_KMAJOR, bool B_KMAJOR>
__global__ __launch_bounds__(GEMM_THREADS, 2) void gemm_xcd_kernel(GemmArgsT<R> p, int tiles_n, int ntiles) {
  __shared__ __attribute__((aligned(16))) R smem[4 * Real<R>::KT * TILE];
#ifdef GPFIT_CLOCK_STAMPS
  const long long t0 = __builtin_amdgcn_s_memtime(), w0 = __builtin_amdgcn_s_memrealtime();
#endif
  gemm_tile_body<R, A_KMAJOR, B_KMAJOR, false, TILE, 2>(p, tiles_n, ntiles, smem);
#ifdef GPFIT_CLOCK_STAMPS
  if (threadIdx.x == 0 && blockIdx.x < 4096) {
    g_gemm_clock[B_KMAJOR ? 1 : 0][blockIdx.x][0] = (long long)__builtin_amdgcn_s_memtime() - t0;
    g_gemm_clock[B_KMAJOR ? 1 : 0][blockIdx.x][1] = (long long)__builtin_amdgcn_s_memrealtime() - w0;
  }
#endif
}

template <typename R, bool A_KMAJOR, bool B_KMAJOR, int EPI>
__global__ __launch_bounds__(GEMM_THREADS, 2) void gemm_epi_kernel(GemmArgsT<R> p, int tiles_n, int ntiles) {
  __shared__ __attribute__((aligned(16))) R smem[4 * Real<R>::KT * TILE];
#ifdef GPFIT_CLOCK_STAMPS
  const long long t0 = __builtin_amdgcn_s_memtime(), w0 = __builtin_amdgcn_s_memrealtime();
#endif
  gemm_tile_body<R, A_KMAJOR, B_KMAJOR, false, TILE, 2, EPI>(p, tiles_n, ntiles, smem);
#ifdef GPFIT_CLOCK_STAMPS
  if (threadIdx.x == 0 && blockIdx.x < 4096 && EPI != 4) {
    g_gemm_clock[B_KMAJOR ? 1 : 0][blockIdx.x][0] = (long long)__builtin_amdgcn_s_memtime() - t0;
    g_gemm_clock[B_KMAJOR ? 1 : 0][blockIdx.x][1] = (long long)__builtin_amdgcn_s_memrealtime() - w0;
  }
#endif
}

template <typename R>
int gemm_pick_tile(const GemmArgsT<R>& a) {
  if (a.k_slabs > 0) return SLAB_TILE;
  if (a.tile == 128 || a.tile == 64 || a.tile == 32) return a.tile;
  auto ntiles = [&](int T) {
    const long tm = (a.M + T - 1) / T, tn = (a.N + T - 1) / T;
    const long nb = (a.M + TILE - 1) / TILE;
    return (a.out_lower ? (long)lower_tile_count((int)nb, TILE / T) : tm * tn) * (a.nptr > 0 ? a.nptr : (a.batch > 0 ? a.batch : 1)) *
           (a.split_k > 1 ? a.split_k : 1);
  };
  static const long t128_min = getenv("GPFIT_T128_MIN") ? atol(getenv("GPFIT_T128_MIN")) : 384;
  static const long t128_tri_min = getenv("GPFIT_T128_TRI_MIN") ? atol(getenv("GPFIT_T128_TRI_MIN")) : 1024;
  const bool batch_tri = a.nptr > 0 && (a.a_tri || a.b_tri);
  if (ntiles(128) >= (batch_tri ? t128_tri_min : t128_min)) return 128;
  static const long t64_min = getenv("GPFIT_T64_MIN") ? atol(getenv("GPFIT_T64_MIN")) : 256;
  static const long t32_dim = getenv("GPFIT_T32_DIM") ? atol(getenv("GPFIT_T32_DIM")) : 1024;
  if (ntiles(64) >= t64_min) return 64;
  return (a.M <= t32_dim && a.N <= t32_dim) ? 32 : 64;
}

constexpr int HALF_OCC_LDS = 17 * 1024;
static void allow_dynamic_lds(const void* fn) {
  static std::mutex mu;
  static std::set<std::pair<const void*, int>> done;
  int device = 0;
  (void)hipGetDevice(&device);
  std::lock_guard<std::mutex> lock(mu);
  if (done.insert({fn, device}).second)
    (void)hipFuncSetAttribute(fn, hipFuncAttributeMaxDynamicSharedMemorySize, HALF_OCC_LDS);
}

static int gemm_stages(int T, bool edge, long blocks) {
  static const int deep_max = getenv("GPFIT_DEEP_MAX") ? atoi(getenv("GPFIT_DEEP_MAX")) : 512;
  return (T == TILE || edge || blocks > deep_max) ? 2 : (T == 64 ? 4 : 8);
}

template <typename R>
static int streamk_first_tile(const GemmArgsT<R>& a, long ntiles) {
  static const bool disabled = getenv("GPFIT_NO_STREAMK") != nullptr;
  if (disabled) return -1;
  static const int sk_min = getenv("GPFIT_SK_MIN_TILES") ? atoi(getenv("GPFIT_SK_MIN_TILES")) : 384;
  if (ntiles < sk_min || (long)a.K < 1024) return -1;
  static const int sk_classes = getenv("GPFIT_SK_CLASSES") ? atoi(getenv("GPFIT_SK_CLASSES")) : 5;
  const bool cls1 = (a.a_tri != 0 && a.b_tri != 0), cls2 = (a.out_lower && a.a_tri == 2 && a.b_tri == 0);
  if ((cls1 && !(sk_classes & 1)) || (cls2 && !(sk_classes & 2))) return -1;
  if (cls1 || cls2) return 0;
  if (!(sk_classes & 4)) return -1;
  if (a.a_tri || a.b_tri) return -1;
  const int tail = (int)(ntiles % SK_SLOTS);
  if (tail == 0 || tail >= 384 || ntiles < SK_SLOTS) return -1;
  return (int)ntiles - tail;
}

template <typename R>
GemmRoute gemm_route(const GemmArgsT<R>& a) {
  GemmRoute r{};
  r.sk_first = -1;
  if (a.M <= 0 || a.N <= 0) return r;
  const int T = r.tile = gemm_pick_tile(a);
  auto refuse = [T](const char* why) {
    GemmRoute e{};
    e.rc = -3; e.error = why; e.tile = T; e.sk_first = -1;
    return e;
  };
  const bool strided = a.batch > 1 && a.nptr <= 0;
  r.tiles_n = (a.N + T - 1) / T;
  r.tiles = a.out_lower ? lower_tile_count((a.M + TILE - 1) / TILE, TILE / T) : ((a.M + T - 1) / T) * r.tiles_n;
  r.edge = (a.M % T) || (a.N % T) || (a.out_lower && (a.M % TILE));

  if (T == TILE && !r.edge && a.nptr <= 0 && a.batch <= 1 && a.split_k <= 1 && !a.half_occ &&
      (a.tile == 0 || a.tile == TILE)) {
    static const long xcd_min = getenv("GPFIT_XCD_MIN_TILES") ? atol(getenv("GPFIT_XCD_MIN_TILES")) : 1536;
    const long tm = a.M / TILE, tn = a.N / TILE, ntiles = a.out_lower ? tm * (tm + 1) / 2 : tm * tn;
    if ((a.reverse & 8) && !(a.out_lower && a.M != a.N) && tm < 32768 && tn < 32768 && ntiles >= xcd_min) r.sched = GEMM_XCD;
    else if ((r.sk_first = streamk_first_tile(a, ntiles)) >= 0) r.sched = GEMM_STREAMK;
  }

  if (a.epi) {
    bool ok = a.split_k <= 1 && a.k_slabs <= 0 && !strided && T == TILE && !(a.M % T) && !(a.N % T) && !a.a_kmajor && !a.half_occ;
    if ((a.epi & 1) && (!a.out_lower || a.M != a.N)) ok = false;
    if ((a.epi & 4) && a.nptr <= 0 && a.aux == nullptr) ok = false;
    if (!((a.epi == 2 && a.b_kmajor) || (a.epi == 1 && !a.b_kmajor) || (a.epi == 4 && a.b_kmajor))) ok = false;
    if (r.sched == GEMM_STREAMK && !(r.sk_first == 0 && a.out_lower && a.M == a.N && a.epi == 2 && a.sumsq != nullptr)) ok = false;
    if (!ok) return refuse("launch_gemm: this launch cannot carry a fused epilogue (gemm_route says so beforehand)");
  }
  constexpr int EPC = 16 / (int)sizeof(R);
  if (a.K % ktile_of<R>() != 0 || (a.lda % EPC) || (a.ldb % EPC))
    return refuse("launch_gemm: K must be a multiple of the K step and lda, ldb multiples of 16 bytes");
  if (a.out_lower && a.M != a.N) return refuse("launch_gemm: out_lower needs a square output");
  if (a.nptr > 0 && (a.nptr > GEMM_MAXB || a.sched || a.split_k > 1))
    return refuse("launch_gemm: a pointer batch holds at most GEMM_MAXB plain problems");
  if (a.k_slabs > 0 &&
      (a.a_tri != 2 || a.b_tri || a.out_lower || a.M != a.K || (a.M % SLAB_TILE) || a.split_k > 1 || a.sched ||
       a.half_occ || strided || (a.tile != 0 && a.tile != SLAB_TILE)))
    return refuse("launch_gemm: k_slabs needs an upper triangular square op(A) on whole 64-tiles and a plain launch");

  r.epi = a.epi;
  if (a.epi & 2) r.sumsq_entries = (r.sched == GEMM_STREAMK ? 33 : 1) * r.tiles;
  r.gx = r.sched == GEMM_XCD ? 0 : (r.sched == GEMM_STREAMK ? r.sk_first : r.tiles);
  if (a.k_slabs > 0) {
    const SlabPlan sp = slab_plan(a.M, a.k_slabs);
    r.gx = sp.items * r.tiles_n;
    r.slabs = sp.live;
  }
  r.gy = a.nptr > 0 ? a.nptr : std::max(a.batch, 1);
  r.gz = a.split_k > 1 ? a.split_k : 1;
  r.stages = gemm_stages(T, r.edge, (long)r.gx * r.gy * r.gz);
  r.half = T == TILE && a.half_occ;
  return r;
}
template GemmRoute gemm_route<double>(const GemmArgsT<double>&);
template GemmRoute gemm_route<float>(const GemmArgsT<float>&);

template <typename R, int T>
static void launch_T(const GemmArgsT<R>& p, const GemmRoute& r, hipStream_t s) {
  const int tn = r.tiles_n, tiles = r.tiles;
  const bool edge = r.edge, deep = r.stages > 2, half = r.half;
  dim3 grid(r.gx, r.gy, r.gz);
  dim3 block(GEMM_THREADS);
  constexpr int DEEP = (T == 128) ? 2 : (T == 64 ? 4 : 8);
#define GP_LAUNCH(AK, BK, ED)                                                                          \
  do {                                                                                                 \
    if (deep) hipLaunchKernelGGL((gemm_mfma_kernel<R, AK, BK, ED, T, (ED ? 2 : DEEP)>), grid, block, 0, s, p, tn, tiles); \
    else if (half) {                                                                                   \
      allow_dynamic_lds(reinterpret_cast<const void*>(gemm_mfma_kernel<R, AK, BK, ED, T, 2>));          \
      hipLaunchKernelGGL((gemm_mfma_kernel<R, AK, BK, ED, T, 2>), grid, block, HALF_OCC_LDS, s, p, tn, tiles); \
    } else hipLaunchKernelGGL((gemm_mfma_kernel<R, AK, BK, ED, T, 2>), grid, block, 0, s, p, tn, tiles); \
  } while (0)
  if (r.epi) {
    if constexpr (T == TILE) {
      const int key = r.epi * 4 + (p.a_kmajor ? 2 : 0) + (p.b_kmajor ? 1 : 0);
      if (key == 2 * 4 + 1) hipLaunchKernelGGL((gemm_epi_kernel<R, false, true, 2>), grid, block, 0, s, p, tn, tiles);
      else if (key == 1 * 4 + 0) hipLaunchKernelGGL((gemm_epi_kernel<R, false, false, 1>), grid, block, 0, s, p, tn, tiles);
      else if (key == 4 * 4 + 1) hipLaunchKernelGGL((gemm_epi_kernel<R, false, true, 4>), grid, block, 0, s, p, tn, tiles);
    }
    return;
  }
  if (p.sched && T == TILE && !edge) {
    switch ((p.a_kmajor ? 2 : 0) | (p.b_kmajor ? 1 : 0)) {
      case 0: hipLaunchKernelGGL((gemm_xcd_kernel<R, false, false>), grid, block, 0, s, p, tn, tiles); break;
      case 1: hipLaunchKernelGGL((gemm_xcd_kernel<R, false, true>), grid, block, 0, s, p, tn, tiles); break;
      case 2: hipLaunchKernelGGL((gemm_xcd_kernel<R, true, false>), grid, block, 0, s, p, tn, tiles); break;
      default: hipLaunchKernelGGL((gemm_xcd_kernel<R, true, true>), grid, block, 0, s, p, tn, tiles); break;
    }
    return;
  }
  const int sel = (p.a_kmajor ? 4 : 0) | (p.b_kmajor ? 2 : 0) | (edge ? 1 : 0);
  switch (sel) {
    case 0: GP_LAUNCH(false, false, false); break;
    case 1: GP_LAUNCH(false, false, true); break;
    case 2: GP_LAUNCH(false, true, false); break;
    case 3: GP_LAUNCH(false, true, true); break;
    case 4: GP_LAUNCH(true, false, false); break;
    case 5: GP_LAUNCH(true, false, true); break;
    case 6: GP_LAUNCH(true, true, false); break;
    case 7: GP_LAUNCH(true, true, true); break;
  }
#undef GP_LAUNCH
}

template <typename R>
int launch_gemm(const GemmArgsT<R>& a, const GemmRoute& route, hipStream_t s) {
  if (route.rc != 0) {
    set_error(route.error);
    return route.rc;
  }
  if (route.tile == 0) return 0;
  if (route.sched == GEMM_XCD) return launch_gemm_xcd(a, route, s);
  if (route.sched != GEMM_STREAMK) return launch_gemm_plain(a, route, s);
  const int rc = launch_gemm_streamk(a, route, s);
  if (rc <= 0) return rc;
  GemmRoute r = route;
  r.stay_data_parallel();
  return launch_gemm_plain(a, r, s);
}

template <typename R>
int launch_gemm_plain(const GemmArgsT<R>& a, const GemmRoute& r, hipStream_t s) {
  GemmArgsT<R> p = a;
  p.batch = r.gy;
  switch (r.tile) {
    case 128: launch_T<R, 128>(p, r, s); break;
    case 64: launch_T<R, 64>(p, r, s); break;
    default: launch_T<R, 32>(p, r, s); break;
  }
  GP_HIP(hipGetLastError());
  return 0;
}

template <typename R>
struct GemmPairT {
  GemmArgsT<R> g[2];
  int tiles[2], tiles_n[2];
};

template <typename R, int T, int NS>
__global__ __launch_bounds__(GEMM_THREADS, (NS > 2 ? 2 : 4)) void gemm_pair_kernel(GemmPairT<R> q) {
  __shared__ __attribute__((aligned(16))) R smem[2 * NS * Real<R>::KT * T];
  const int w = blockIdx.z;
  const GemmArgsT<R>& p = q.g[w];
  if ((int)blockIdx.x >= q.tiles[w] || (int)blockIdx.y >= p.batch) return;
  if (p.b_kmajor) gemm_tile_body<R, false, true, false, T, NS>(p, q.tiles_n[w], q.tiles[w], smem);
  else gemm_tile_body<R, false, false, false, T, NS>(p, q.tiles_n[w], q.tiles[w], smem);
}

template <typename R>
static GemmRoute pair_member_route(const GemmArgsT<R>& a) {
  const GemmRoute none{};
  if (a.nptr <= 0 || a.epi || a.k_slabs > 0 || a.half_occ || a.a_kmajor || (a.M % 64) || (a.N % 64)) return none;
  const GemmRoute r = gemm_route(a);
  return (r.rc == 0 && !r.edge && (r.tile == 32 || r.tile == 64)) ? r : none;
}

template <typename R>
GemmRoute gemm_pair_shape(const GemmArgsT<R>& a, const GemmArgsT<R>& b) {
  static const bool off = getenv("GPFIT_NO_PAIR") != nullptr;
  static const bool no64 = getenv("GPFIT_NO_PAIR64") != nullptr;
  GemmRoute h{};
  h.sk_first = -1;
  const GemmRoute ra = pair_member_route(a), rb = pair_member_route(b);
  if (off || ra.tile == 0 || ra.tile != rb.tile || (no64 && ra.tile == 64)) {
    h.rc = -3;
    h.error = "launch_gemm_pair: the two problems cannot share a launch (gemm_pair_shape says so beforehand)";
    return h;
  }
  h.tile = ra.tile;
  h.tiles = ra.tiles * ra.gy + rb.tiles * rb.gy;
  h.stages = gemm_stages(h.tile, false, h.tiles);
  h.gx = std::max(ra.tiles, rb.tiles);
  h.gy = std::max(ra.gy, rb.gy);
  h.gz = 2;
  return h;
}
template GemmRoute gemm_pair_shape<double>(const GemmArgsT<double>&, const GemmArgsT<double>&);
template GemmRoute gemm_pair_shape<float>(const GemmArgsT<float>&, const GemmArgsT<float>&);

template <typename R>
int launch_gemm_pair(const GemmArgsT<R>& a, const GemmArgsT<R>& b, const GemmRoute& h, hipStream_t s) {
  if (h.rc != 0) {
    set_error(h.error);
    return h.rc;
  }
  static_assert(sizeof(GemmPairT<R>) <= 4096, "kernel arguments are limited to 4 KiB");
  const int T = h.tile;
  GemmPairT<R> q;
  for (int w = 0; w < 2; ++w) {
    q.g[w] = w == 0 ? a : b;
    GemmArgsT<R>& p = q.g[w];
    p.batch = p.nptr;
    q.tiles_n[w] = p.N / T;
    q.tiles[w] = p.out_lower ? lower_tile_count(p.M / TILE, TILE / T) : (p.M / T) * (p.N / T);
  }
  const dim3 grid(h.gx, h.gy, h.gz), block(GEMM_THREADS);
  const bool deep = h.stages > 2;
  if (T == 32 && deep) hipLaunchKernelGGL((gemm_pair_kernel<R, 32, 8>), grid, block, 0, s, q);
  else if (T == 32) hipLaunchKernelGGL((gemm_pair_kernel<R, 32, 2>), grid, block, 0, s, q);
  else if (deep) hipLaunchKernelGGL((gemm_pair_kernel<R, 64, 4>), grid, block, 0, s, q);
  else hipLaunchKernelGGL((gemm_pair_kernel<R, 64, 2>), grid, block, 0, s, q);
  GP_HIP(hipGetLastError());
  return 0;
// ... 19 lines not shown
```

gaussian_processes_amd/csrc/gemm_core.h:

```cpp
#pragma once
#include "common.h"

#include <cstdint>
#include <vector>

namespace gpfit {

typedef double v4d __attribute__((ext_vector_type(4)));
typedef double v2d __attribute__((ext_vector_type(2)));
typedef float v4f __attribute__((ext_vector_type(4)));

constexpr int GEMM_THREADS = 256;

template <typename R> struct Real;
template <> struct Real<double> {
  using acc_t = v4d;
  using vec_t = v2d;
  static constexpr int EPC = 2, KT = 16;
  static __device__ __forceinline__ acc_t mfma(double a, double b, acc_t c) {
    return __builtin_amdgcn_mfma_f64_16x16x4f64(a, b, c, 0, 0, 0);
  }
  static __device__ __forceinline__ int crow(int lane, int r) { return (lane >> 4) + 4 * r; }
  static __device__ __forceinline__ int swz(int k) { return (((k >> 1) & 7) << 1) | ((k & 1) << 4); }
};
// ... 41 lines not shown
      if (!EDGE || ((valid >> i) & 1u)) r[i] = *reinterpret_cast<const V*>(base + off[i]);
      else r[i] = V{};
    }
  }
  __device__ __forceinline__ void advance() { base += step; }
};

template <typename R, bool KMAJOR, int T>
__device__ __forceinline__ void tile_sstore(const typename Real<R>::vec_t (&r)[T / 32], R* __restrict__ S, int tid) {
  using V = typename Real<R>::vec_t;
  constexpr int EPC = Real<R>::EPC;
#pragma unroll
  for (int i = 0; i < T / 32; ++i) {
    const int c = tid + GEMM_THREADS * i;
    if (KMAJOR) {
      const int k = c / (T / EPC), x = EPC * (c % (T / EPC));
      *reinterpret_cast<V*>(S + k * T + (x ^ Real<R>::swz(k))) = r[i];
    } else {
      const int x = c >> 3, k = EPC * (c & 7);
#pragma unroll
      for (int e = 0; e < EPC; ++e) S[(k + e) * T + (x ^ Real<R>::swz(k + e))] = r[i][e];
    }
  }
}

template <typename R, bool A_KMAJOR, bool B_KMAJOR, int T>
__device__ __forceinline__ void gemm_mainloop_regstage(const R* __restrict__ A, int64_t lda, const R* __restrict__ B,
                                                       int64_t ldb, int M, int N, int row0, int col0, int kbeg,
                                                       int kend, R* smem, typename Real<R>::acc_t (&acc)[T / 32][T / 32]) {
  using V = typename Real<R>::vec_t;
  constexpr int MI = T / 32, WT = T / 2, KT = Real<R>::KT, LT = KT * T;
  const int tid = threadIdx.x;
  const int lane = tid & 63, wave = tid >> 6;
  const int wm = wave >> 1, wn = wave & 1;
  const int fr = lane & 15, fk = lane >> 4;
  V ra[MI], rb[MI];

  if (kbeg >= kend) return;
  TileSrc<R, A_KMAJOR, true, T> sa;
  TileSrc<R, B_KMAJOR, true, T> sb;
  sa.init(A, lda, row0, kbeg, M, tid);
  sb.init(B, ldb, col0, kbeg, N, tid);
  sa.load(ra);
  sb.load(rb);
  __syncthreads();
  tile_sstore<R, A_KMAJOR, T>(ra, smem, tid);
  tile_sstore<R, B_KMAJOR, T>(rb, smem + LT, tid);
  __syncthreads();
  if (kbeg + KT < kend) {
    sa.advance();
    sb.advance();
    sa.load(ra);
    sb.load(rb);
  }
  int buf = 0;
  for (int k0 = kbeg; k0 < kend; k0 += KT) {
    const bool more = (k0 + KT) < kend;
    const bool more2 = (k0 + 2 * KT) < kend;
    const R* As = smem + buf * 2 * LT;
    const R* Bs = As + LT;
    R* Sn = smem + (buf ^ 1) * 2 * LT;
#pragma unroll
    for (int kk = 0; kk < KT / 4; ++kk) {
      const int krow = kk * 4 + fk;
      const int sw = Real<R>::swz(krow);
      R a[MI], b[MI];
#pragma unroll
      for (int i = 0; i < MI; ++i) {
        a[i] = As[krow * T + ((wm * WT + i * 16 + fr) ^ sw)];
        b[i] = Bs[krow * T + ((wn * WT + i * 16 + fr) ^ sw)];
      }
#pragma unroll
      for (int mi = 0; mi < MI; ++mi)
#pragma unroll
        for (int ni = 0; ni < MI; ++ni) acc[mi][ni] = Real<R>::mfma(a[mi], b[ni], acc[mi][ni]);
      if (kk == KT / 8 && more) {
        tile_sstore<R, A_KMAJOR, T>(ra, Sn, tid);
        tile_sstore<R, B_KMAJOR, T>(rb, Sn + LT, tid);
        if (more2) {
          sa.advance();
          sb.advance();
          sa.load(ra);
          sb.load(rb);
        }
      }
    }
    __syncthreads();
    buf ^= 1;
  }
}

template <typename R, int T> struct LdsImage {
  static constexpr int EPC = Real<R>::EPC, KT = Real<R>::KT;
  static constexpr int SWK = (EPC == 2 ? 1 : 3) & (T / 16 - 1);
  template <bool KMAJOR> static __device__ __forceinline__ int at(int x, int k) {
    if (KMAJOR) return k * T + (x ^ (16 * (k & SWK)));
    return x * KT + ((((k / EPC) ^ ((x >> 1) & 7))) * EPC) + (k % EPC);
  }
};

template <typename R, bool KMAJOR, int T> struct TileDma {
  static constexpr int MI = T / 32, EPC = Real<R>::EPC, KT = Real<R>::KT;
  const char* base;
  int64_t step;
  uint32_t voff[MI];
  int q0;

  __device__ __forceinline__ void init(const R* __restrict__ P, int64_t ld, int x0, int k0, int wave, int lane) {
    base = reinterpret_cast<const char*>(KMAJOR ? P + (int64_t)k0 * ld + x0 : P + (int64_t)x0 * ld + k0);
    step = (KMAJOR ? (int64_t)KT * ld : (int64_t)KT) * (int64_t)sizeof(R);
    q0 = wave * MI;
#pragma unroll
    for (int i = 0; i < MI; ++i) {
      const int pch = (q0 + i) * 64 + lane;
      int64_t e;
      if (KMAJOR) {
        constexpr int CPR = T / EPC;
        const int k = pch / CPR, xs = (pch % CPR) * EPC;
        e = (int64_t)k * ld + (xs ^ (16 * (k & LdsImage<R, T>::SWK)));
      } else {
        const int x = pch >> 3, j = (pch & 7) ^ ((x >> 1) & 7);
        e = (int64_t)x * ld + j * EPC;
      }
      voff[i] = (uint32_t)(e * (int64_t)sizeof(R));
    }
  }
  __device__ __forceinline__ void issue(uint32_t image) const {
    const __amdgpu_buffer_rsrc_t rs = __builtin_amdgcn_make_buffer_rsrc(const_cast<char*>(base), 0, -1, 0x00020000);
#pragma unroll
    for (int i = 0; i < MI; ++i)
      __builtin_amdgcn_raw_ptr_buffer_load_lds(
          rs, (__attribute__((address_space(3))) void*)(uintptr_t)(image + (uint32_t)(q0 + i) * 1024u), 16, voff[i], 0, 0, 0);
  }
  __device__ __forceinline__ void issue_one(uint32_t image, int i) const {
    const __amdgpu_buffer_rsrc_t rs = __builtin_amdgcn_make_buffer_rsrc(const_cast<char*>(base), 0, -1, 0x00020000);
    __builtin_amdgcn_raw_ptr_buffer_load_lds(
        rs, (__attribute__((address_space(3))) void*)(uintptr_t)(image + (uint32_t)(q0 + i) * 1024u), 16, voff[i], 0, 0, 0);
  }
  __device__ __forceinline__ void advance() { base += step; }
};

template <int N> __device__ __forceinline__ void dma_wait_barrier() {
  asm volatile("s_waitcnt vmcnt(%0) lgkmcnt(0)\n\ts_barrier" ::"n"(N) : "memory");
}

template <typename R, bool A_KMAJOR, bool B_KMAJOR, bool EDGE, int T, int ABL = 0, int NS = 2>
__device__ __forceinline__ void gemm_mainloop(const R* __restrict__ A, int64_t lda, const R* __restrict__ B,
                                              int64_t ldb, int M, int N, int row0, int col0, int kbeg, int kend,
                                              R* smem, typename Real<R>::acc_t (&acc)[T / 32][T / 32],
                                              bool kdesc = false) {
  if constexpr (EDGE) {
    gemm_mainloop_regstage<R, A_KMAJOR, B_KMAJOR, T>(A, lda, B, ldb, M, N, row0, col0, kbeg, kend, smem, acc);
    return;
  } else {
    constexpr int MI = T / 32, WT = T / 2, KT = Real<R>::KT, LT = KT * T, NKK = KT / 4;
    constexpr int D = NS - 1;
    constexpr int OPS = 2 * MI;
    static_assert(NS >= 2 && (D - 1) * OPS < 64, "vmcnt is a 6-bit counter");
    using Img = LdsImage<R, T>;
    const int tid = threadIdx.x;
    const int lane = tid & 63, wave = __builtin_amdgcn_readfirstlane(tid >> 6);
    const int wm = wave >> 1, wn = wave & 1;
    const int fr = lane & 15, fk = lane >> 4;
    row0 = __builtin_amdgcn_readfirstlane(row0);
    col0 = __builtin_amdgcn_readfirstlane(col0);
    kbeg = __builtin_amdgcn_readfirstlane(kbeg);
    kend = __builtin_amdgcn_readfirstlane(kend);
    if (kbeg >= kend) return;
    const int ntile = (kend - kbeg) / KT;

    TileDma<R, A_KMAJOR, T> da;
    TileDma<R, B_KMAJOR, T> db;
    da.init(A, lda, row0, kdesc ? kend - KT : kbeg, wave, lane);
    db.init(B, ldb, col0, kdesc ? kend - KT : kbeg, wave, lane);
    if (kdesc) {
      da.step = -da.step;
      db.step = -db.step;
    }
    const uint32_t lds0 = (uint32_t)(uintptr_t)smem;
    constexpr uint32_t LTB = LT * sizeof(R);
    auto issue = [&](int stage) {
      const uint32_t img = lds0 + (uint32_t)stage * 2u * LTB;
      da.issue(img);
      db.issue(img + LTB);
      da.advance();
      db.advance();
    };

    __syncthreads();
#pragma unroll
    for (int t = 0; t < D; ++t)
      if (t < ntile) issue(t);
    if (ntile >= D) dma_wait_barrier<(D - 1) * OPS>();
    else dma_wait_barrier<0>();

    R fa[2][MI], fb[2][MI];
    auto frag = [&](const R* S, int kk, R (&a)[MI], R (&b)[MI]) {
      const int k = kk * 4 + fk;
#pragma unroll
      for (int i = 0; i < MI; ++i) {
        a[i] = S[Img::template at<A_KMAJOR>(wm * WT + i * 16 + fr, k)];
        b[i] = S[LT + Img::template at<B_KMAJOR>(wn * WT + i * 16 + fr, k)];
      }
    };
    frag(smem, 0, fa[0], fb[0]);

    int cs = 0;
    for (int s = 0; s < ntile; ++s) {
      const bool more = (s + 1) < ntile;
      const int nx = (cs + 1 == NS) ? 0 : cs + 1;
      const R* Sc = smem + cs * 2 * LT;
      const R* Sn = smem + nx * 2 * LT;
      if (s + D < ntile && !(ABL & 2)) issue((cs + D) % NS);
#pragma unroll
      for (int kk = 0; kk < NKK; ++kk) {
        const int cur = kk & 1, nxt = cur ^ 1;
        if (kk + 1 < NKK) {
          frag(Sc, kk + 1, fa[nxt], fb[nxt]);
        } else if (more) {
          if (!(ABL & 1)) {
            if (s + D < ntile) dma_wait_barrier<(D - 1) * OPS>();
            else dma_wait_barrier<0>();
          }
          frag(Sn, 0, fa[nxt], fb[nxt]);
        }
#pragma unroll
        for (int mi = 0; mi < MI; ++mi)
#pragma unroll
          for (int ni = 0; ni < MI; ++ni) acc[mi][ni] = Real<R>::mfma(fa[cur][mi], fb[cur][ni], acc[mi][ni]);
      }
      cs = nx;
    }
  }
}

template <typename R, int T, typename F>
__device__ __forceinline__ void for_each_acc(const typename Real<R>::acc_t (&acc)[T / 32][T / 32], int row0,
                                             int col0, F&& f) {
  const int lane = threadIdx.x & 63, wave = threadIdx.x >> 6;
  const int wm = wave >> 1, wn = wave & 1;
#pragma unroll
  for (int mi = 0; mi < T / 32; ++mi)
#pragma unroll
    for (int ni = 0; ni < T / 32; ++ni)
#pragma unroll
      for (int r = 0; r < 4; ++r) {
        const int row = row0 + wm * (T / 2) + mi * 16 + Real<R>::crow(lane, r);
        const int col = col0 + wn * (T / 2) + ni * 16 + (lane & 15);
        f(row, col, acc[mi][ni][r]);
      }
}

__device__ __host__ inline void tri_tile(int t, int& ti, int& tj) {
  int i = (int)((sqrt(8.0 * (double)t + 1.0) - 1.0) * 0.5);
  while ((i + 1) * (i + 2) / 2 <= t) ++i;
  while (i * (i + 1) / 2 > t) --i;
  ti = i;
  tj = t - i * (i + 1) / 2;
}

__device__ __host__ inline void lower_tile(int t, int r, int& ti, int& tj) {
  int bi, rem;
  tri_tile(t / (r * r), bi, rem);
  const int start = r * r * (bi * (bi + 1) / 2);
  const int v = t - start;
  const int w = (bi + 1) * r;
  ti = bi * r + v / w;
  tj = v % w;
}
__host__ __device__ inline int lower_tile_count(int nblocks, int r) { return r * r * (nblocks * (nblocks + 1) / 2); }

__host__ __device__ __forceinline__ void gemm_walk_tile(int b, int walk, bool lower, int r, int tiles_n, int ntiles,
                                                        int& ti, int& tj) {
  const int bid = (walk & 1) ? (ntiles - 1 - b) : b;
  if (lower && (walk & 2) && r == 1) {
    const int nt = tiles_n;
    int j = (int)((2.0 * nt + 1.0 - sqrt((2.0 * nt + 1.0) * (2.0 * nt + 1.0) - 8.0 * (double)bid)) * 0.5);
    while (j > 0 && (long)j * nt - (long)j * (j - 1) / 2 > bid) --j;
    while ((long)(j + 1) * nt - (long)(j + 1) * j / 2 <= bid) ++j;
    tj = j;
    ti = j + (bid - (j * nt - j * (j - 1) / 2));
  } else if (lower) {
    lower_tile(bid, r, ti, tj);
  } else if (walk & 2) {
    const int tiles_m = ntiles / tiles_n;
    tj = bid / tiles_m;
    ti = bid % tiles_m;
  } else {
    ti = bid / tiles_n;
    tj = bid % tiles_n;
  }
}

struct KRange { int beg, end; };
__host__ __device__ __forceinline__ KRange gemm_tile_k_range(int a_tri, int b_tri, int K, int row0, int col0, int T) {
  int kbeg = 0, kend = K;
  if (a_tri == 1) kend = kend < row0 + T ? kend : row0 + T;
  if (a_tri == 2) kbeg = kbeg > row0 ? kbeg : row0;
  if (b_tri == 1) kbeg = kbeg > col0 ? kbeg : col0;
  if (b_tri == 2) kend = kend < col0 + T ? kend : col0 + T;
  return {kbeg, kend};
}

constexpr int SK_SLOTS = 512;
struct SkTile {
  int row0, col0, kbeg, ksteps;
  int prefix;
};
struct SkHostPlan {
  std::vector<SkTile> tiles;
  int total = 0, blocks = 0, per_block = 0;
  std::vector<int> fix_tile;
  std::vector<int> fix_ptr;
  std::vector<int> fix_slot;
};
template <typename R> int streamk_plan_host(const GemmArgsT<R>& a, int first, SkHostPlan& plan);
template <typename R> int xcd_plan_host(const GemmArgsT<R>& a, std::vector<int>& table);

}
```

gaussian_processes_amd/csrc/kernels.h:

```cpp
#pragma once
#include "common.h"
#include "lbfgs1d.h"

namespace gpfit {

struct Theta {
  double sigma0, eps0x, eps0y, logbeta, logrho, amp;
  double eb, er;
};

template <typename R>
struct GroupPrepT {
  int n_units, n, np;
  const int* pix_host[GEMM_MAXB / 2];
  int* pix[GEMM_MAXB / 2];
  int d[GEMM_MAXB / 2];
  int* info[GEMM_MAXB / 2];
  const R* m[GEMM_MAXB / 2];
  R* mpad[GEMM_MAXB / 2];
};
struct GroupCollectT {
  int n_units;
  const double* scal[GEMM_MAXB / 2];
  const int* info[GEMM_MAXB / 2];
  double* scal_host[GEMM_MAXB / 2];
  int* info_host[GEMM_MAXB / 2];
};
template <typename R>
int launch_group_prepare(const GroupPrepT<R>& g, hipStream_t s);
int launch_group_collect(const GroupCollectT& g, hipStream_t s);

template <typename R>
struct LeafBatchT {
  const R* A[GEMM_MAXB];
  R* L[GEMM_MAXB];
  R* Li[GEMM_MAXB];
  int* info[GEMM_MAXB];
  int64_t lda, ldl, ldi;
  int info_base;
  int n;
};
template <typename R> int launch_chol_leaf_batch(const LeafBatchT<R>& bt, hipStream_t s);

template <typename R>
int launch_localker(const Theta& th, const int* pix, int d, int dp, int n_rows, int n_cols, R* C, int64_t ldc,
                    R* dC, hipStream_t s);
template <typename R>
int launch_gather(const R* X, int64_t ldx, int n, const int* pix, int d, int dp, int np, R* Xt, int64_t ldt, R* Xm,
                  int64_t ldm, hipStream_t s);
template <typename R>
int launch_qvec(const R* Xt, const R* XCt, int64_t ld, int dp, int n, int np, double s0sq, R* Kvec, R* q,
                hipStream_t s);
template <typename R>
int launch_pack_lower(const R* src, int64_t lds, int n, R* dst, int64_t ldd, int np, hipStream_t s);
template <typename R> int launch_symmetrize(R* A, int64_t lda, int n, hipStream_t s);
template <typename R> int launch_logdet(const R* L, int64_t ldl, int n, double* out, hipStream_t s);
template <typename R> int launch_logdet_pair(const R* L0, double* out0, const R* L1, double* out1, int64_t ldl, int n, hipStream_t s);
template <typename R>
int launch_frob_lower(const R* T, int64_t ldt, int np, double* out, double* partial, hipStream_t s);
template <typename R> int launch_trmv_lower(const R* L, int64_t ldl, int np, const R* x, R* y, hipStream_t s);
template <typename R>
int launch_trmv_lower_t(const R* L, int64_t ldl, int np, const R* x, R* z, double* partial, hipStream_t s);
template <typename R>
int launch_gemv_sub(const R* M, int64_t ldm, int rows, int cols, const R* x, const R* y, R* out, hipStream_t s);
template <typename R>
int launch_gemv_t_sub(const R* M, int64_t ldm, int rows, int cols, const R* x, const R* y, R* out, double* partial,
                      hipStream_t s);
template <typename R>
int launch_frob_tiles(const R* T, int64_t ldt, int rows, int cols, int lower, double* partial, hipStream_t s);
int launch_demote_block(const double* src, int64_t lds, float* dst, int64_t ldd, int rows, int cols, hipStream_t s);
template <typename R> int launch_dot(const R* x, const R* y, int n, double* out, hipStream_t s);

template <typename R>
int launch_moments(const R* Kvec, const R* q, const R* Cos, int64_t ldc, const R* V, int64_t ldv, const R* m,
                   const R* r, int n, double A, double lambda0, R* lam_m, R* lam_var, R* f, R* wl, double* scal,
                   double* part, int* ticket, hipStream_t s);

template <typename R>
int launch_adjoint(const R* W, const R* Cos, int64_t ld, const R* b, const R* q, int n, int np, R* Aout,
                   double* upart, double* vpart, double* sumA_part, hipStream_t s);
template <typename R>
int launch_adjoint_reduce(const double* upart, const double* vpart, const double* sumA_part, int ntile,
                          int ntile_tri, const R* q, const R* wl, int n, int np, R* tvec, double* uq,
                          double* scal_out, hipStream_t s);
template <typename R>
int launch_rowscale_add(R* Y, int64_t ldy, const R* Xm, int64_t ldm, const R* t, int np, int dp, hipStream_t s,
                        double scale = 1.0);
template <typename RI, typename RO>
int launch_reduce_slices(const RI* src, int64_t slice_stride, int nslice, RO* dst, int64_t count, hipStream_t s);
template <typename R>
int launch_reduce_slabs(const R* src, int64_t slab_stride, int nslab, int slab_rows, R* dst, int rows, int cols, hipStream_t s);
template <typename R>
int launch_reduce_slices_sym(const R* src, int64_t slice_stride, int nslice, R* dst, int n, hipStream_t s);
template <typename R>
int launch_metric_contract(const Theta& th, const int* pix, int d, int n_rows, int n_cols, const R* C, int64_t ldc,
                           const R* M, int64_t ldm, double* grad5, double* part ,
                           int* ticket , hipStream_t s);
int launch_frob_finish(const double* partial, int nt, double* out, hipStream_t s);
template <typename R> int launch_add_diag(R* A, int64_t lda, int n, double v, hipStream_t s);
template <typename R> int launch_scale_copy(R* dst, const R* src, int n, double alpha, hipStream_t s);
template <typename R>
int launch_axpby_block(R* dst, int64_t ldd, const R* src, int64_t lds, int rows, int cols, double a, double b,
                       hipStream_t s);

int launch_adjoint_rect(const double* W, int64_t ldw, const double* Cos, int64_t ldc, const double* q1,
                        const double* q2, int n1, int n2, int np1, int np2, double* Aout, int64_t lda, double* upart,
                        double* vpart, double* tile_sum, const double* extra1, double* t1, double* t2, double* uq1,
                        double* uq2, double* scal3, hipStream_t s);

int launch_nd_utility(const double* sigma2, const double* mu, int64_t nstar, const double* r, int nr, double* U,
                      hipStream_t s);

int launch_pad_copy(const double* src, int64_t lds, int rows, int cols, double* dst, int64_t ldd, int prow,
                    int pcol, hipStream_t s);
int launch_symmetrize_avg(double* A, int64_t lda, int n, hipStream_t s);
int launch_dk_sigma0(const double* Cos, int64_t ldc, const double* q1, const double* q2, int n1, int n2,
                     double s0, double* dK, int64_t ldk, hipStream_t s);
int launch_dq(const double* Xt, const double* XDt, int64_t ld, int dp, int n, const double* q, double* dq,
              double* h, hipStream_t s);
int launch_dk_metric(double* H, int64_t ldh, const double* Cos, int64_t ldc, const double* q1, const double* q2,
                     const double* dq1, const double* dq2, int n1, int n2, hipStream_t s);
int launch_fill(double* x, int64_t n, double v, hipStream_t s);

int launch_proj_moments(const double* Bp, const double* Kb, const double* aV, int64_t ld, int nb, const double* mb,
                        const double* Kvec, const double* r, int n, double A, double lambda0, double* lam_m,
                        double* lam_var, double* f, double* gm, double* gv, double* part, double* out3, hipStream_t s);
int launch_proj_ga(const double* Kb, const double* aV, int64_t ld, int nb, int n, int np, const double* gm,
                   const double* gv, const double* mb, double* Ga, hipStream_t s);
int launch_proj_gkb(const double* Bp, int64_t ld, int nb, int n, int np, const double* gv, double* GaKi, hipStream_t s);
int launch_proj_gktb(const double* Ki, const double* P1, const double* P2, int64_t ld, int nb, const double* b, double* G,
                     hipStream_t s);
int launch_proj_trace(const double* A, int64_t lda, int n, double* out, hipStream_t s);
int launch_estep_proj_rows(const double* a, int64_t lda, int nb, const double* mb, const double* f, const double* r,
                           int n, int nrows, double A, double* sv, double* u, hipStream_t s);
int launch_estep_proj_scale(const double* aL, int64_t ldal, int nb, int n, int nrows, const double* sv, const double* u,
                            double* Y, double* aLp , int64_t ld, int npc, double* part, hipStream_t s);
int launch_estep_proj_moments(const double* Z, int64_t ld, int nb, const double* z1, const double* kv0, int n,
                              double* lam_m, double* lam_var, hipStream_t s);

int launch_estep_prep(const double* f, const double* r, const double* m, int n, int np, double A, double* sv,
                      double* rhs, hipStream_t s);
int launch_estep_build(const double* K, int64_t ldk, int n, int np, const double* sv, double* Mb, double* SK,
                       double* Kl, int64_t ld, hipStream_t s);
int launch_symv_lower(const double* A, int64_t lda, int n, const double* x, double* y, hipStream_t s);
int launch_unpack_sym(const double* src, int64_t lds, int n, double* dst, int64_t ldd, hipStream_t s);
int launch_unpack_tri(const double* src, int64_t lds, int n, double* dst, int64_t ldd, hipStream_t s);
int launch_fparam(const double* lam_m, const double* lam_var, const double* r, int n, double A, int closed_form,
                  double lambda0_in, double* f, double* out, hipStream_t s);
int launch_fparam_lbfgs(const double* lam_m, const double* lam_var, const double* r, int n, double logA0,
                        int lambda0_mode, double lambda0_fixed, const Lbfgs1dConfig& cfg, double* f, double* out,
                        hipStream_t s);

constexpr int CHAIN_MAX_STEPS = 1024;
constexpr int CHAIN_REC = 12;
enum ChainRecSlot {
  CR_LBFGS = 0,
  CR_INFO = 9,
  CR_RAN = 10,
  CR_A = 11,
};
struct ChainBlock {
  double logA;
  double lambda0;
  int stop, pad;
  double rec[CHAIN_MAX_STEPS][CHAIN_REC];
};
struct ChainGate {
  const int* stop;
  const int* info;
  __device__ __forceinline__ bool open() const { return *stop == 0 && *info == 0; }
};
constexpr int CHAIN_MAXU = GEMM_MAXB / 2;
template <typename T>
struct PerUnit {
  T v[CHAIN_MAXU];
  __host__ __device__ __forceinline__ T operator[](int u) const { return v[u]; }
};
struct ChainGroupT {
  int n_units, n, nrows, npc, kmax;
  int64_t ld;
  PerUnit<int> nb;
  PerUnit<const double*> a, aL, L, r, kv0;
  PerUnit<int64_t> lda, ldal, ldl, ldv;
  PerUnit<double*> m, f, V, lam_m, lam_var;
  PerUnit<double> logA0, lambda0;
  PerUnit<ChainBlock*> blk;
  PerUnit<int*> info;
  PerUnit<double*> rec_host;
  PerUnit<double*> sv, u, t2, z1, z, mo, Y, Lp, Vw, part, aLp, Zm, W, Li, trmv_part;
};
int launch_chain_init_group(const ChainGroupT& g, int n_steps, hipStream_t s);
int launch_estep_proj_rows_chain_group(const ChainGroupT& g, int step, hipStream_t s);
int launch_estep_proj_scale_group(const ChainGroupT& g, hipStream_t s);
int launch_chain_info_group(const ChainGroupT& g, int step, hipStream_t s);
int launch_chain_copy_group(const ChainGroupT& g, hipStream_t s);
int launch_unpack_sym_chain_group(const ChainGroupT& g, hipStream_t s);
int launch_estep_proj_moments_chain_group(const ChainGroupT& g, hipStream_t s);
int launch_fparam_lbfgs_chain_group(const ChainGroupT& g, int step, int lambda0_mode, const Lbfgs1dConfig& cfg, hipStream_t s);
int launch_chain_collect_group(const ChainGroupT& g, int n_steps, hipStream_t s);
int launch_estep_prep_chain(const double* f, const double* r, const double* m, int n, int np, ChainBlock* blk, int step,
                            int* info, double* sv, double* rhs, hipStream_t s);
int launch_estep_full_moments_chain(ChainGate g, const double* m_new, const double* Vw, int64_t ld, const double* kv0,
                                    int n, double* lam_m, double* lam_var, hipStream_t s);
int launch_pack_lower_group(int n_units, PerUnit<const double*> src, PerUnit<int64_t> lds, PerUnit<int> n, PerUnit<double*> dst,
                            int64_t ldd, int np, hipStream_t s);
int launch_add_diag_group(int n_units, PerUnit<double*> A, int64_t lda, int n, double v, hipStream_t s);
int launch_reduce_slices_group(int n_units, PerUnit<double*> src, int64_t slice_stride, int nslice, PerUnit<double*> dst,
                               int64_t count, hipStream_t s);
int launch_trmv_lower_group(int n_units, PerUnit<double*> L, int64_t ldl, int np, PerUnit<double*> x, PerUnit<double*> y,
                            hipStream_t s);
int launch_trmv_lower_t_group(int n_units, PerUnit<double*> L, int64_t ldl, int np, PerUnit<double*> x, PerUnit<double*> z,
                              PerUnit<double*> partial, hipStream_t s);

struct ClosurePrepT {
  int n_units, nb, cap_max;
  PerUnit<const int*> pix_host;
  PerUnit<int*> pix, info;
  PerUnit<int> d, nk, cap;
  PerUnit<const double*> m_b;
  PerUnit<double*> mpad, bv, wl;
};
int launch_closure_prepare(const ClosurePrepT& g, hipStream_t s);
int launch_zero3_group(int n_units, PerUnit<double*> a, PerUnit<double*> b, PerUnit<double*> c, int64_t count, hipStream_t s);
int launch_pad_copy_group(int n_units, PerUnit<const double*> src, PerUnit<int64_t> lds, int rows, PerUnit<int> cols,
                          PerUnit<double*> dst, int64_t ldd, int prow, int pcol, hipStream_t s);
int launch_symmetrize_group(int n_units, PerUnit<double*> A, int64_t lda, int n, hipStream_t s);
int launch_symmetrize_avg_group(int n_units, PerUnit<double*> A, int64_t lda, PerUnit<int> n, hipStream_t s);
int launch_logdet_pair_group(int n_units, PerUnit<const double*> L0, PerUnit<double*> out0, PerUnit<const double*> L1,
                             PerUnit<double*> out1, int64_t ldl, PerUnit<int> n, hipStream_t s);
int launch_symv_lower_group(int n_units, PerUnit<double*> A, int64_t lda, int n, PerUnit<double*> x, PerUnit<double*> y,
                            hipStream_t s);
int launch_dot_group(int n_units, PerUnit<double*> x, PerUnit<double*> y, int n, PerUnit<double*> out, hipStream_t s);
int launch_proj_trace_group(int n_units, PerUnit<double*> A, int64_t lda, PerUnit<int> n, PerUnit<double*> out, hipStream_t s);
struct ProjGroupT {
  int n_units, n, np, nb;
  int64_t ld;
  PerUnit<const double*> r;
  PerUnit<double> A, lambda0;
  PerUnit<double*> am, Kb, aV, mb, Kvec, lam_m, lam_var, f, gm, gv, part, out3;
  PerUnit<double*> Ga, GaKi;
  PerUnit<double*> Ki, P1, P2, bvec, G;
};
int launch_proj_moments_group(const ProjGroupT& g, hipStream_t s);
int launch_proj_ga_group(const ProjGroupT& g, hipStream_t s);
int launch_proj_gkb_group(const ProjGroupT& g, hipStream_t s);
int launch_proj_gktb_group(const ProjGroupT& g, hipStream_t s);

}
```

include/gpfit_mi355x.h:

```cpp
#ifndef GPFIT_MI355X_H
#define GPFIT_MI355X_H

#include <stdint.h>

#ifdef __cplusplus
extern "C" {
#endif

#define GPFIT_VERSION 100

int gpfit_version(void);
const char* gpfit_last_error(void);

int gpfit_dgemm(void* stream, int a_kmajor, int b_kmajor, int M, int N, int K, double alpha,
                const double* A, int64_t lda, const double* B, int64_t ldb, double beta, double* C,
                int64_t ldc, int out_lower, int a_tri, int b_tri);
int gpfit_dgemm_ex(void* stream, int a_kmajor, int b_kmajor, int M, int N, int K, double alpha,
                   const double* A, int64_t lda, const double* B, int64_t ldb, double beta, double* C,
                   int64_t ldc, int out_lower, int a_tri, int b_tri, int walk, int tile);

typedef struct gpfit_ctx gpfit_ctx;
int gpfit_ctx_create(int device, int64_t n_max, int64_t d_max, int64_t d_full_max, gpfit_ctx** out);
void gpfit_ctx_destroy(gpfit_ctx* ctx);

int gpfit_check_limits(const double* theta, const double* lower, const double* upper);

int gpfit_localker_mask(const double* theta, int n_rows, int n_cols, uint8_t* mask_host, int64_t* d_out);

int gpfit_localker(gpfit_ctx* ctx, void* stream, const double* theta, int n_rows, int n_cols,
                   const uint8_t* mask_host, int64_t d, double* C, double* dC);

int gpfit_acosker(gpfit_ctx* ctx, void* stream, double sigma0, const double* x1, int64_t ld1, int64_t n1,
                  const double* x2, int64_t ld2, int64_t n2, int64_t d, const double* C, int64_t ldC,
                  const double* dC, double* K, int64_t ldk, double* dK);

int gpfit_acosker_pullback(gpfit_ctx* ctx, void* stream, double sigma0, const double* x1, int64_t ld1,
                           int64_t n1, const double* x2, int64_t ld2, int64_t n2, int64_t d, const double* C,
                           int64_t ldC, const double* W, int64_t ldw, const double* t1_extra, double* M_out,
                           int64_t ldm, double* out_host);

int gpfit_acosker_diag(gpfit_ctx* ctx, void* stream, double sigma0, const double* x1, int64_t ld1,
                       int64_t n1, int64_t d, const double* C, int64_t ldC, const double* dC, double* Kvec,
                       double* dKvec);

int gpfit_fit_eval(gpfit_ctx* ctx, void* stream, const double* theta, const double* lower,
                   const double* upper, int n_rows, int n_cols, const double* X, int64_t ldx, int64_t N,
                   const double* r, const double* m, const double* V, int64_t ldv, double logA,
                   double lambda0, int want_grad, double* out_host, double* lam_m, double* lam_var,
                   double* f);

int gpfit_fit_eval_finish(gpfit_ctx* ctx, double* out_host);

int gpfit_fit_eval_batch(gpfit_ctx* const* ctxs, int n_units, void* stream, const double* theta,
                         const double* lower, const double* upper, int n_rows, int n_cols,
                         const double* const* X, int64_t ldx, int64_t N, const double* const* r,
                         const double* const* m, const double* const* V, int64_t ldv, const double* logA,
                         const double* lambda0, int want_grad, double* out_host, int* rc_out);
int gpfit_fit_eval_batch_f32(gpfit_ctx* const* ctxs, int n_units, void* stream, const double* theta,
                             const double* lower, const double* upper, int n_rows, int n_cols,
                             const float* const* X, int64_t ldx, int64_t N, const float* const* r,
                             const float* const* m, const float* const* V, int64_t ldv, const double* logA,
                             const double* lambda0, int want_grad, double* out_host, int* rc_out);

int gpfit_grad_pullback(gpfit_ctx* ctx, void* stream, const double* theta, int n_rows, int n_cols,
                        const double* X, int64_t ldx, int64_t N, const double* W, int64_t ldw,
                        const double* gvec, double* out_host);

int gpfit_fit_eval_projected(gpfit_ctx* ctx, void* stream, const double* theta, const double* lower,
                             const double* upper, int n_rows, int n_cols, const double* X, int64_t ldx, int64_t N,
                             const double* r, const double* B, int64_t ldb, int64_t n_kept, const double* m_b,
                             const double* V_b, int64_t ldvb, double logA, double lambda0, double* out_host);

int gpfit_fit_eval_sparse(gpfit_ctx* ctx, void* stream, const double* theta, const double* lower, const double* upper,
                          int n_rows, int n_cols, const double* X, int64_t ldx, int64_t N, const double* Xtilde,
                          int64_t ldxt, int64_t Ntilde, const double* r, const double* B, int64_t ldb, int64_t n_kept,
                          const double* m_b, const double* V_b, int64_t ldvb, double logA, double lambda0,
                          double* out_host);

#define GPFIT_FIT_EVAL_SPARSE_MAX_UNITS 16
int gpfit_fit_eval_sparse_batch(gpfit_ctx* const* ctxs, int n_units, void* stream, const double* theta,
                                const double* lower, const double* upper, int n_rows, int n_cols,
                                const double* const* X, int64_t ldx, int64_t N, const double* const* Xtilde,
                                int64_t ldxt, int64_t Ntilde, const double* const* r, const double* const* B,
                                const int64_t* ldb, const int64_t* n_kept, const double* const* m_b,
                                const double* const* V_b, const int64_t* ldvb, const double* logA,
                                const double* lambda0, double* out_host, int* rc_out);

int gpfit_potrf(gpfit_ctx* ctx, void* stream, const double* A, int64_t lda, int64_t n, double* L, int64_t ldl,
                double* Linv, int64_t ldi, double* logdet_host, int* info_host);

int gpfit_potrf_append(gpfit_ctx* ctx, void* stream, double* L, int64_t ldl, double* Linv, int64_t ldi, int64_t n,
                       const double* kcol, double* logdet_inout_host, int* info_host);

int gpfit_estep(gpfit_ctx* ctx, void* stream, const double* K, int64_t ldk, int64_t N, const double* r,
                const double* m, const double* f, double logA, double* m_new, double* V_new, int64_t ldv);

int gpfit_estep_projected(gpfit_ctx* ctx, void* stream, const double* a, int64_t lda, const double* aL, int64_t ldal,
                          const double* L, int64_t ldl, int64_t N, int64_t nb, const double* r, const double* m,
                          const double* f, double logA, double* m_new, double* V_new, int64_t ldv, const double* kv0,
                          double* lam_m_out, double* lam_var_out);

int gpfit_fparam_eval(gpfit_ctx* ctx, void* stream, const double* lam_m, const double* lam_var,
                      const double* r, int64_t N, double logA, int closed_form_lambda0, double lambda0_in,
                      double* f_out, double* out_host);

int gpfit_fparam_lbfgs(gpfit_ctx* ctx, void* stream, const double* lam_m, const double* lam_var,
                       const double* r, int64_t N, double logA0, int lambda0_mode, double lambda0_fixed,
                       int max_iter, int history_size, double lr, double tol_grad, double tol_change,
                       double* f_out, double* out_host);
int gpfit_fparam_lbfgs_host(const double* lam_m, const double* lam_var, const double* r, int64_t N,
                            double logA0, int lambda0_mode, double lambda0_fixed, int max_iter,
                            int history_size, double lr, double tol_grad, double tol_change, double* f_out,
                            double* out_host);

#define GPFIT_ESTEP_CHAIN_MAX_STEPS 1024
int gpfit_estep_chain(gpfit_ctx* ctx, void* stream, const double* a, int64_t lda, const double* aL, int64_t ldal,
                      const double* L, int64_t ldl, int64_t N, int64_t nb, const double* r, const double* kv0,
                      double* m, double* f, double* V, int64_t ldv, double* lam_m, double* lam_var, double logA0,
                      int lambda0_mode, double lambda0_fixed, int n_steps, int max_iter, int history_size, double lr,
                      double tol_grad, double tol_change, double* rec_host);

int gpfit_estep_chain_full(gpfit_ctx* ctx, void* stream, const double* K, int64_t ldk, int64_t N, const double* r,
                           const double* kv0, double* m, double* f, double* V, int64_t ldv, double* lam_m,
                           double* lam_var, double logA0, int lambda0_mode, double lambda0_fixed, int n_steps,
                           int max_iter, int history_size, double lr, double tol_grad, double tol_change,
                           double* rec_host);

#define GPFIT_ESTEP_CHAIN_MAX_UNITS 16
int gpfit_estep_chain_batch(gpfit_ctx* const* ctxs, int n_units, void* stream, const double* const* a,
                            const int64_t* lda, const double* const* aL, const int64_t* ldal, const double* const* L,
                            const int64_t* ldl, int64_t N, const int64_t* nb, const double* const* r,
                            const double* const* kv0, double* const* m, double* const* f, double* const* V,
                            const int64_t* ldv, double* const* lam_m, double* const* lam_var, const double* logA0,
                            int lambda0_mode, const double* lambda0_fixed, int n_steps, int max_iter, int history_size,
                            double lr, double tol_grad, double tol_change, double* rec_host);

int gpfit_nd_utility(void* stream, const double* sigma2, const double* mu, int64_t nstar, const double* r,
                     int nr, double* U);

int gpfit_set_profile(gpfit_ctx* ctx, int on);
int gpfit_get_profile(gpfit_ctx* ctx, double* out16);
int gpfit_get_phases(gpfit_ctx* ctx, double* out8);
double gpfit_last_enqueue_ms(gpfit_ctx* ctx);

int gpfit_fit_eval_f32(gpfit_ctx* ctx, void* stream, const double* theta, const double* lower,
                       const double* upper, int n_rows, int n_cols, const float* X, int64_t ldx, int64_t N,
                       const float* r, const float* m, const float* V, int64_t ldv, double logA, double lambda0,
                       int want_grad, double* out_host, float* lam_m, float* lam_var, float* f);

int gpfit_probe_mfma_f64(void* stream, double* scratch, int blocks, int iters);
int gpfit_probe_stream_copy(void* stream, const double* in, double* out, int64_t n_doubles);

typedef struct gpfit_dev_gemm_args {
  const void* A;
  const void* B;
  void* C;
  int64_t lda, ldb, ldc;
  int64_t sA, sB, sC;
  double alpha, beta;
  void* sk_ws;
  void* aux;
  double* sumsq;
  const void* const* Ap;
  const void* const* Bp;
  void* const* Cp;
  void* const* auxp;
  double* const* sumsqp;
  int32_t M, N, K;
  int32_t a_kmajor, b_kmajor, out_lower, a_tri, b_tri;
  int32_t batch;
  int32_t split_k;
  int32_t tile;
  int32_t walk;
  int32_t epi;
  int32_t nptr;
  int32_t k_slabs;
} gpfit_dev_gemm_args;

typedef struct gpfit_dev_gemm_route_t {
  int32_t rc;
  int32_t tile;
  int32_t sk_first;
  int32_t xcd;
  int32_t stages;
  int32_t half_occ;
  int32_t edge;
  int32_t epi;
  int32_t sumsq_entries;
  int32_t blocks;
  int32_t pair;
  int32_t slabs;
} gpfit_dev_gemm_route_t;

int gpfit_dev_gemm_route(int is_f32, const gpfit_dev_gemm_args* args, const gpfit_dev_gemm_args* pair_args,
                         gpfit_dev_gemm_route_t* out);
int64_t gpfit_dev_gemm_plan(int is_f32, const gpfit_dev_gemm_args* args, int kind, int32_t* out, int64_t cap);
int gpfit_dev_gemm(void* stream, int is_f32, const gpfit_dev_gemm_args* args, const gpfit_dev_gemm_args* pair_args);
int gpfit_dev_ctx_copy(gpfit_ctx* ctx, const char* name, int64_t offset, void* dev, int64_t bytes, int to_ctx);
int gpfit_dev_ctx_fill(gpfit_ctx* ctx, const char* name, int byte);

#ifdef __cplusplus
}
#endif
#endif
```

Measured before the change: 36.65 fits/s.

## Fuse Cholesky leaf factorization with following 128-sized TRSM/merge product

```diff
diff --git a/gaussian_processes_amd/_lib.py b/gaussian_processes_amd/_lib.py
--- a/gaussian_processes_amd/_lib.py
+++ b/gaussian_processes_amd/_lib.py
@@ -75,6 +75,7 @@
     "gpfit_dev_gemm_route": (i32, [i32, ctypes.POINTER(DevGemmArgs), ctypes.POINTER(DevGemmArgs), ctypes.POINTER(DevGemmRoute)]),
     "gpfit_dev_gemm_plan": (i64, [i32, ctypes.POINTER(DevGemmArgs), i32, ctypes.POINTER(ctypes.c_int32), i64]),
     "gpfit_dev_gemm": (i32, [vp, i32, ctypes.POINTER(DevGemmArgs), ctypes.POINTER(DevGemmArgs)]),
+    "gpfit_dev_leaf_replicas": (i32, [i32, i32]),
     "gpfit_dev_ctx_copy": (i32, [vp, ctypes.c_char_p, i64, vp, i64, i32]),
     "gpfit_dev_ctx_fill": (i32, [vp, ctypes.c_char_p, i32]),
 }
diff --git a/gaussian_processes_amd/csrc/api_dev.hip b/gaussian_processes_amd/csrc/api_dev.hip
--- a/gaussian_processes_amd/csrc/api_dev.hip
+++ b/gaussian_processes_amd/csrc/api_dev.hip
@@ -162,6 +162,8 @@
                 : gpfit::run<double>((hipStream_t)stream, *args, pair_args);
 }
 
+int gpfit_dev_leaf_replicas(int nb, int cus) { return gpfit::leaf_replicas(nb, cus); }
+
 int gpfit_dev_ctx_copy(gpfit_ctx* ctx, const char* name, int64_t offset, void* dev, int64_t bytes, int to_ctx) {
   if (!ctx || !name || !dev || offset < 0 || bytes < 0 || ctx->pend.active) return -3;
   gpfit::DeviceGuard guard(ctx->device);
diff --git a/gaussian_processes_amd/csrc/chol_leaf_reg.hip b/gaussian_processes_amd/csrc/chol_leaf_reg.hip
--- a/gaussian_processes_amd/csrc/chol_leaf_reg.hip
+++ b/gaussian_processes_amd/csrc/chol_leaf_reg.hip
@@ -257,23 +257,37 @@
   }
 }
 
+
+constexpr int RL_PANEL = RL * RPS, RL_DIAG = 16 * RPS;
+constexpr int RL_LDS_ELEMS = 2 * RL_PANEL + 5 * RL_DIAG + 4;
 template <typename R>
-__global__ __launch_bounds__(RL_THREADS, 2) void chol_leaf_reg_kernel(LeafBatchT<R> bt) {
-  const R* __restrict__ A = bt.A[blockIdx.x];
-  R* __restrict__ L = bt.L[blockIdx.x];
-  R* __restrict__ Linv = bt.Li[blockIdx.x];
-  int* __restrict__ info = bt.info[blockIdx.x];
-  const int64_t lda = bt.lda, ldl = bt.ldl, ldi = bt.ldi;
-  const int info_base = bt.info_base;
+struct LeafLds {
+  R (&Rawb)[1][RL_PANEL];
+  R (&Lpb)[1][RL_PANEL];
+  R (&Dbuf)[2][RL_DIAG];
+  R (&Dgb)[2][RL_DIAG];
+  R (&Sx)[RL_DIAG];
+  unsigned& b2_arrivals;
+  static __device__ __forceinline__ LeafLds carve(R* m) {
+    return {*reinterpret_cast<R (*)[1][RL_PANEL]>(m), *reinterpret_cast<R (*)[1][RL_PANEL]>(m + RL_PANEL),
+            *reinterpret_cast<R (*)[2][RL_DIAG]>(m + 2 * RL_PANEL), *reinterpret_cast<R (*)[2][RL_DIAG]>(m + 2 * RL_PANEL + 2 * RL_DIAG),
+            *reinterpret_cast<R (*)[RL_DIAG]>(m + 2 * RL_PANEL + 4 * RL_DIAG), *reinterpret_cast<unsigned*>(m + RL_LDS_ELEMS - 4)};
+  }
+};
+
+template <typename R>
+__device__ __forceinline__ void chol_leaf_body(const R* __restrict__ A, R* __restrict__ L, R* __restrict__ Linv, int* __restrict__ info,
+                                               const int64_t lda, const int64_t ldl, const int64_t ldi, const int info_base,
+                                               bool report, const LeafLds<R> lds) {
   using Acc = typename Real<R>::acc_t;
   using V = typename Real<R>::vec_t;
   constexpr int EPC = Real<R>::EPC;
-  __shared__ __attribute__((aligned(16))) R Rawb[1][RL * RPS];
-  __shared__ __attribute__((aligned(16))) R Lpb[1][RL * RPS];
-  __shared__ __attribute__((aligned(16))) R Dbuf[2][16 * RPS];
-  __shared__ __attribute__((aligned(16))) R Dgb[2][16 * RPS];
-  __shared__ __attribute__((aligned(16))) R Sx[16 * RPS];
-  __shared__ unsigned b2_arrivals;
+  R (&Rawb)[1][RL_PANEL] = lds.Rawb;
+  R (&Lpb)[1][RL_PANEL] = lds.Lpb;
+  R (&Dbuf)[2][RL_DIAG] = lds.Dbuf;
+  R (&Dgb)[2][RL_DIAG] = lds.Dgb;
+  R (&Sx)[RL_DIAG] = lds.Sx;
+  unsigned& b2_arrivals = lds.b2_arrivals;
   const int tid = threadIdx.x, lane = tid & 63;
   const int wave = __builtin_amdgcn_readfirstlane(tid >> 6);
   const int fr = lane & 15;
@@ -312,7 +326,7 @@
       LEAF_STAMP(nx, 1);
       static_for_pivots<R, 0>(v, yh, myr, first_bad, li, 16 * nx);
       LEAF_STAMP(nx, 2);
-      if (lane == 0 && first_bad != 0) atomicCAS(info, 0, info_base + first_bad);
+      if (report && lane == 0 && first_bad != 0) atomicCAS(info, 0, info_base + first_bad);
       {
         R* drow = Dbuf[nx & 1] + li * RPS + lg;
 #pragma unroll
@@ -377,7 +391,7 @@
         pivot_block(nx, lane_o);
       }
     }
-    return;
+    __builtin_amdgcn_endpgm();
   }
 
   Acc acc[RL_SLOTS];
@@ -473,6 +487,44 @@
 }
 
 template <typename R>
+__global__ __launch_bounds__(RL_THREADS, 2) void chol_leaf_reg_kernel(LeafBatchT<R> bt) {
+  __shared__ __attribute__((aligned(16))) R Rawb[1][RL_PANEL];
+  __shared__ __attribute__((aligned(16))) R Lpb[1][RL_PANEL];
+  __shared__ __attribute__((aligned(16))) R Dbuf[2][RL_DIAG];
+  __shared__ __attribute__((aligned(16))) R Dgb[2][RL_DIAG];
+  __shared__ __attribute__((aligned(16))) R Sx[RL_DIAG];
+  __shared__ unsigned b2_arrivals;
+  const int b = blockIdx.x;
+  chol_leaf_body<R>(bt.A[b], bt.L[b], bt.Li[b], bt.info[b], bt.lda, bt.ldl, bt.ldi, bt.info_base, true,
+                    LeafLds<R>{Rawb, Lpb, Dbuf, Dgb, Sx, b2_arrivals});
+}
+
+template <typename R>
+__global__ __launch_bounds__(RL_THREADS, 2) void chol_leaf_fused_kernel(LeafFusedT<R> ft) {
+  constexpr int T = 32, NS = 8, TILES_N = RL / T, NTILES = TILES_N * TILES_N;
+  __shared__ __attribute__((aligned(16))) R smem[2 * NS * Real<R>::KT * T];
+  static_assert(sizeof(smem) >= RL_LDS_ELEMS * sizeof(R), "the leaf's buffers are carved from the operand stages");
+  const int nb = ft.leaf.n;
+  const int chain = (int)blockIdx.x % nb, g = (int)blockIdx.x / nb;
+  const bool takes_part = (ft.need >> chain) & 1u;
+  if (!takes_part && g > 0) return;
+  const LeafBatchT<R>& bt = ft.leaf;
+  chol_leaf_body<R>(bt.A[chain], bt.L[chain], bt.Li[chain], bt.info[chain], bt.lda, bt.ldl, bt.ldi, bt.info_base, g == 0,
+                    LeafLds<R>::carve(smem));
+  if (!takes_part) return;
+  asm volatile("s_waitcnt vmcnt(0)" ::: "memory");
+  __syncthreads();
+  const int problem = __popc(ft.need & ((1u << chain) - 1u));
+  const int G = ft.replicas;
+#pragma unroll 1
+  for (int j = 0; j * G < NTILES; ++j) {
+    const TileAt at{j * G + ((j & 1) ? G - 1 - g : g), problem, 0};
+    if (ft.prod.b_kmajor) gemm_tile_body<R, false, true, false, T, NS>(ft.prod, TILES_N, NTILES, smem, at);
+    else gemm_tile_body<R, false, false, false, T, NS>(ft.prod, TILES_N, NTILES, smem, at);
+  }
+}
+
+template <typename R>
 int launch_chol_leaf_batch(const LeafBatchT<R>& bt, hipStream_t s) {
   if (bt.n <= 0 || bt.n > GEMM_MAXB) {
     set_error("launch_chol_leaf_batch: 1 .. GEMM_MAXB blocks per launch");
@@ -483,7 +535,26 @@
   return 0;
 }
 
+template <typename R>
+int launch_chol_leaf_fused(const LeafFusedT<R>& ft, hipStream_t s) {
+  static_assert(sizeof(LeafFusedT<R>) <= 4096, "kernel arguments are limited to 4 KiB");
+  const GemmArgsT<R>& p = ft.prod;
+  const int G = ft.replicas;
+  const uint32_t all = ft.leaf.n >= 32 ? 0xffffffffu : ((1u << ft.leaf.n) - 1u);
+  if (ft.leaf.n <= 0 || ft.leaf.n > GEMM_MAXB || (G != 2 && G != 4 && G != 8) || ft.need == 0 || (ft.need & ~all) ||
+      p.nptr != __builtin_popcount(ft.need) || p.M != RL || p.N != RL || p.K != RL || p.a_kmajor || p.out_lower || p.epi ||
+      p.split_k > 1 || p.k_slabs > 0 || p.sched != nullptr) {
+    set_error("launch_chol_leaf_fused: not a 128-sized plain product per chain behind the leaf");
+    return -3;
+  }
+  hipLaunchKernelGGL(chol_leaf_fused_kernel<R>, dim3(ft.leaf.n * G), dim3(RL_THREADS), 0, s, ft);
+  GP_HIP(hipGetLastError());
+  return 0;
+}
+
 template int launch_chol_leaf_batch<double>(const LeafBatchT<double>&, hipStream_t);
 template int launch_chol_leaf_batch<float>(const LeafBatchT<float>&, hipStream_t);
-
-}
+template int launch_chol_leaf_fused<double>(const LeafFusedT<double>&, hipStream_t);
+template int launch_chol_leaf_fused<float>(const LeafFusedT<float>&, hipStream_t);
+
+}
diff --git a/gaussian_processes_amd/csrc/context.h b/gaussian_processes_amd/csrc/context.h
--- a/gaussian_processes_amd/csrc/context.h
+++ b/gaussian_processes_amd/csrc/context.h
@@ -108,6 +108,7 @@
   ProfScope(hipStream_t s, double flops, int kind);
   ~ProfScope();
 };
+void prof_add_flops(double flops, int kind);
 template <typename R> double gemm_flops(const GemmArgsT<R>& g, int tile);
 
 template <typename R>
@@ -123,6 +124,9 @@
   int side_min = 0;
 };
 template <typename R>
-int potrf_lockstep(const CholBatchT<R>& B, int r0, int n, uint32_t need, Lane lane, uint32_t halves = 0);
+struct LeafBehind { GemmArgsT<R> prod; uint32_t chains; int replicas; };
+template <typename R>
+int potrf_lockstep(const CholBatchT<R>& B, int r0, int n, uint32_t need, Lane lane, uint32_t halves = 0,
+                   const LeafBehind<R>* behind = nullptr);
 
 }
diff --git a/gaussian_processes_amd/csrc/fit.hip b/gaussian_processes_amd/csrc/fit.hip
--- a/gaussian_processes_amd/csrc/fit.hip
+++ b/gaussian_processes_amd/csrc/fit.hip
@@ -52,6 +52,10 @@
   double ms[4] = {0, 0, 0, 0}, fl[4] = {0, 0, 0, 0}, cnt[4] = {0, 0, 0, 0};
   double big_ms = 0, big_fl = 0;
   for (auto& r : c->prof) {
+    if (!r.a) {
+      fl[r.kind] += r.flops;
+      continue;
+    }
     float t = 0.f;
     (void)hipEventElapsedTime(&t, r.a, r.b);
     if (r.kind == 0 && r.flops > big_fl) { big_fl = r.flops; big_ms = t; }
@@ -81,6 +85,10 @@
     (void)hipEventRecord(b, s);
     g_prof->prof.push_back({a, b, flops, kind});
   }
+}
+
+void prof_add_flops(double flops, int kind) {
+  if (g_prof) g_prof->prof.push_back({nullptr, nullptr, flops, kind});
 }
 
 template <typename R>
@@ -213,8 +221,23 @@
 template int product<float>(Lane, Dims, double, const Operand<float>&, const Operand<float>&, const Output<float>&, int,
                             Epilogue<float>*);
 
-template <typename R>
-int potrf_lockstep(const CholBatchT<R>& B, int r0, int n, uint32_t need, Lane lane, uint32_t halves) {
+static int leaf_fuse_replicas(int nb) {
+  static const bool off = getenv("GPFIT_NO_LEAF_FUSE") != nullptr || getenv("GPFIT_NO_BATCH") != nullptr;
+  if (off) return 0;
+  constexpr int MAXDEV = 64;
+  static int cus[MAXDEV];
+  int device = 0;
+  if (hipGetDevice(&device) != hipSuccess || device < 0 || device >= MAXDEV) return 0;
+  if (cus[device] == 0) {
+    int v = 0;
+    if (hipDeviceGetAttribute(&v, hipDeviceAttributeMultiprocessorCount, device) != hipSuccess || v <= 0) v = -1;
+    cus[device] = v;
+  }
+  return leaf_replicas(nb, cus[device]);
+}
+
+template <typename R>
+int potrf_lockstep(const CholBatchT<R>& B, int r0, int n, uint32_t need, Lane lane, uint32_t halves, const LeafBehind<R>* behind) {
   const int64_t ld = B.ld;
   const hipStream_t s = lane.s;
   const uint32_t all = (B.nb >= 32) ? 0xffffffffu : ((1u << B.nb) - 1u);
@@ -228,7 +251,8 @@
   };
   if (n == TILE) {
     ProfScope ps(s, 0.0, 1);
-    LeafBatchT<R> bt{};
+    LeafFusedT<R> ft{};
+    LeafBatchT<R>& bt = ft.leaf;
     bt.n = B.nb;
     for (int b = 0; b < B.nb; ++b) {
       bt.A[b] = B.A[b] + off(r0, r0); bt.L[b] = B.L[b] + off(r0, r0); bt.Li[b] = B.Li[b] + off(r0, r0);
@@ -236,14 +260,33 @@
     }
     bt.lda = bt.ldl = bt.ldi = ld;
     bt.info_base = r0;
-    return launch_chol_leaf_batch(bt, s);
+    if (!behind) return launch_chol_leaf_batch(bt, s);
+    ft.prod = behind->prod;
+    ft.need = behind->chains;
+    ft.replicas = behind->replicas;
+    if (gemm_logging()) {
+      const GemmArgsT<R>& g = ft.prod;
+      fprintf(stderr, "[gpfit gemm] M %d N %d K %d atri %d btri %d lower %d nb %d tile %d ak %d bk %d epi %d flops %.6e", g.M, g.N, g.K,
+              g.a_tri, g.b_tri, g.out_lower, g.nptr, 32, g.a_kmajor, g.b_kmajor, g.epi, gemm_flops(g, 32));
+      gemm_log_tail("", g, "");
+      fprintf(stderr, " leaf_fused %d\n", ft.replicas);
+    }
+    if (g_prof) prof_add_flops(gemm_flops(ft.prod, 32), 3);
+    return launch_chol_leaf_fused(ft, s);
   }
   const int k = n / TILE;
   const int n1 = ((k + 1) / 2) * TILE, n2 = n - n1;
   const int r1 = r0 + n1;
-  GP_TRY(potrf_lockstep<R>(B, r0, n1, all, lane));
-  GP_TRY(product(lane, {n2, n1, n1}, 1.0, plain(blk(all, B.A, r1, r0)), trans(tril(blk(all, B.Li, r0, r0))),
-                 into(blk(all, B.L, r1, r0)), walk(W_TRSM)));
+  const int replicas = (n == 2 * TILE) ? leaf_fuse_replicas(B.nb) : 0;
+  const Dims trsm{n2, n1, n1};
+  const Operand<R> A21 = plain(blk(all, B.A, r1, r0)), Li11t = trans(tril(blk(all, B.Li, r0, r0)));
+  if (replicas) {
+    const LeafBehind<R> lb{batch_args(lane, trsm, 1.0, A21, Li11t, into(blk(all, B.L, r1, r0)), walk(W_TRSM)), all, replicas};
+    GP_TRY(potrf_lockstep<R>(B, r0, n1, all, lane, 0u, &lb));
+  } else {
+    GP_TRY(potrf_lockstep<R>(B, r0, n1, all, lane));
+    GP_TRY(product(lane, trsm, 1.0, A21, Li11t, into(blk(all, B.L, r1, r0)), walk(W_TRSM)));
+  }
   const Operand<R> L21 = plain(blk(all, B.L, r1, r0)), L21t = trans(blk(all, B.L, r1, r0));
   const Output<R> A22 = into_lower(blk(all, B.A, r1, r1), 1.0);
   const Operand<R> L21n = plain(blk(need, B.L, r1, r0)), Li11 = plain(tril(blk(need, B.Li, r0, r0)));
@@ -286,18 +329,29 @@
     }
   }
   if (!merged) GP_TRY(product(lane, syrk, -1.0, L21, L21t, A22));
+  const Dims merge2{n2, n1, n2};
+  const Operand<R> Li22 = plain(tril(blk(need, B.Li, r1, r1))), tmp_in = plain(blk(need, B.Tmp, r1, r0));
+  const Output<R> Li21 = into(blk(need, B.Li, r1, r0));
+  auto tmp_ready = [&]() -> int {
+    if (joined) GP_HIP(hipStreamWaitEvent(s, joined, 0));
+    else if (!merged) GP_TRY(product(lane, merge1, 1.0, L21n, Li11, tmp, walk(W_TMP)));
+    return 0;
+  };
+  if (need && replicas) {
+    GP_TRY(tmp_ready());
+    const LeafBehind<R> lb{batch_args(lane, merge2, -1.0, Li22, tmp_in, Li21, walk(W_MERGE)), need, replicas};
+    return potrf_lockstep<R>(B, r1, n2, need | halves, lane, 0u, &lb);
+  }
   GP_TRY(potrf_lockstep<R>(B, r1, n2, need | halves, lane));
   if (need) {
-    if (joined) GP_HIP(hipStreamWaitEvent(s, joined, 0));
-    else if (!merged) GP_TRY(product(lane, merge1, 1.0, L21n, Li11, tmp, walk(W_TMP)));
-    GP_TRY(product(lane, {n2, n1, n2}, -1.0, plain(tril(blk(need, B.Li, r1, r1))), plain(blk(need, B.Tmp, r1, r0)),
-                   into(blk(need, B.Li, r1, r0)), walk(W_MERGE)));
-  }
-  return 0;
-}
-
-template int potrf_lockstep<double>(const CholBatchT<double>&, int, int, uint32_t, Lane, uint32_t);
-template int potrf_lockstep<float>(const CholBatchT<float>&, int, int, uint32_t, Lane, uint32_t);
+    GP_TRY(tmp_ready());
+    GP_TRY(product(lane, merge2, -1.0, Li22, tmp_in, Li21, walk(W_MERGE)));
+  }
+  return 0;
+}
+
+template int potrf_lockstep<double>(const CholBatchT<double>&, int, int, uint32_t, Lane, uint32_t, const LeafBehind<double>*);
+template int potrf_lockstep<float>(const CholBatchT<float>&, int, int, uint32_t, Lane, uint32_t, const LeafBehind<float>*);
 
 template <typename R>
 struct TwoSidedBufs { R* Q; const R* Li; R *W, *Z, *H; const R* L; int64_t ld; int min_split; };
diff --git a/gaussian_processes_amd/csrc/gemm.hip b/gaussian_processes_amd/csrc/gemm.hip
--- a/gaussian_processes_amd/csrc/gemm.hip
+++ b/gaussian_processes_amd/csrc/gemm.hip
@@ -7,128 +7,6 @@
 #include <utility>
 
 namespace gpfit {
-
-template <typename R, bool A_KMAJOR, bool B_KMAJOR, bool EDGE, int T, int NS>
-__device__ __forceinline__ bool gemm_tile_compute(const GemmArgsT<R>& p, int tiles_n, int ntiles, R* smem,
-                                                  typename Real<R>::acc_t (&acc)[T / 32][T / 32], int& ti, int& tj,
-                                                  int& row0, int& col0, R*& C) {
-  constexpr int KT = Real<R>::KT;
-
-  int slab = 0, slab_tiles = 0;
-  const bool slabbed = (T == SLAB_TILE) && p.k_slabs > 0;
-  if (slabbed) {
-    const SlabPlan sp = slab_plan(p.M, p.k_slabs);
-    slab_item(sp, (int)blockIdx.x / tiles_n, ti, slab);
-    tj = (int)blockIdx.x % tiles_n;
-    slab_tiles = sp.ks;
-  } else if (p.sched != nullptr) {
-    const int e = p.sched[blockIdx.x];
-    if (e < 0) return false;
-    ti = e >> 16;
-    tj = e & 0xffff;
-  } else {
-    gemm_walk_tile((int)blockIdx.x, p.reverse, p.out_lower != 0, TILE / T, tiles_n, ntiles, ti, tj);
-  }
-  row0 = ti * T;
-  col0 = tj * T;
-  const int b = blockIdx.y, z = blockIdx.z;
-  const R* A;
-  const R* B;
-  if (p.nptr > 0) {
-    A = p.Ap[b];
-    B = p.Bp[b];
-    C = p.Cp[b];
-  } else {
-    A = p.A + (int64_t)b * p.sA;
-    B = p.B + (int64_t)b * p.sB;
-    C = p.C + (int64_t)b * p.sC;
-  }
-
-  const KRange kr = gemm_tile_k_range(p.a_tri, p.b_tri, p.K, row0, col0, T);
-  int kbeg = kr.beg, kend = kr.end;
-  if (slabbed) {
-    kbeg = max(kbeg, slab * slab_tiles * T);
-    kend = min(kend, (slab + 1) * slab_tiles * T);
-    C += (int64_t)slab * p.sC;
-  } else if (p.split_k > 1) {
-    const int steps = max(0, kend - kbeg) / KT;
-    const int per = (steps + p.split_k - 1) / p.split_k;
-    const int s0 = min(steps, z * per), s1 = min(steps, (z + 1) * per);
-    kend = kbeg + s1 * KT;
-    kbeg = kbeg + s0 * KT;
-    C += (int64_t)z * p.sC;
-  }
-
-#pragma unroll
-  for (int i = 0; i < T / 32; ++i)
-#pragma unroll
-    for (int j = 0; j < T / 32; ++j) acc[i][j] = acc_zero<R>();
-
-  gemm_mainloop<R, A_KMAJOR, B_KMAJOR, EDGE, T, 0, NS>(A, p.lda, B, p.ldb, p.M, p.N, row0, col0, kbeg, kend, smem, acc,
-                                                       (p.reverse & 4) != 0);
-  return true;
-}
-
-template <typename R, bool A_KMAJOR, bool B_KMAJOR, bool EDGE, int T, int NS, int EPI = 0>
-__device__ __forceinline__ void gemm_tile_body(const GemmArgsT<R>& p, int tiles_n, int ntiles, R* smem) {
-  typename Real<R>::acc_t acc[T / 32][T / 32];
-  int ti, tj, row0, col0;
-  R* C;
-  if (!gemm_tile_compute<R, A_KMAJOR, B_KMAJOR, EDGE, T, NS>(p, tiles_n, ntiles, smem, acc, ti, tj, row0, col0, C)) return;
-
-  const R alpha = (R)p.alpha, beta = (p.split_k > 1 || (T == SLAB_TILE && p.k_slabs > 0)) ? (R)0 : (R)p.beta;
-  const int64_t ldc = p.ldc;
-  const int M = p.M, N = p.N;
-  if constexpr (EPI != 0) {
-    constexpr int epi = EPI;
-    R* __restrict__ D = p.nptr > 0 ? p.auxp[blockIdx.y] : p.aux;
-    double* __restrict__ sumsq = p.nptr > 0 ? p.sumsqp[blockIdx.y] : p.sumsq;
-    double ss = 0.0;
-    for_each_acc<R, T>(acc, row0, col0, [&](int row, int col, R v) {
-      if (EDGE && !(row < M && col < N)) return;
-      R o = alpha * v;
-      R* c = C + (int64_t)row * ldc + col;
-      if (epi & 4) {
-        R* dd = D + (int64_t)row * ldc + col;
-        const R d0 = *dd;
-        o += d0;
-        *dd = o + d0;
-      } else if (beta != (R)0) {
-        o += beta * (*c);
-      }
-      if (epi & 1) {
-        if (row >= col) *c = o;
-        if (row > col) C[(int64_t)col * ldc + row] = o;
-      } else {
-        *c = o;
-      }
-      if (epi & 2) ss += (double)o * (double)o;
-    });
-    if (epi & 2) {
-#pragma unroll
-      for (int o = 32; o > 0; o >>= 1) ss += __shfl_down(ss, o);
-      double* red = reinterpret_cast<double*>(smem);
-      __syncthreads();
-      if ((threadIdx.x & 63) == 0) red[threadIdx.x >> 6] = ss;
-      __syncthreads();
-      if (threadIdx.x == 0)
-        sumsq[p.out_lower ? (int64_t)ti * (ti + 1) / 2 + tj : (int64_t)ti * tiles_n + tj] = (red[0] + red[1]) + (red[2] + red[3]);
-    }
-    return;
-  }
-  if (beta == (R)0) {
-    for_each_acc<R, T>(acc, row0, col0, [&](int row, int col, R v) {
-      if (!EDGE || (row < M && col < N)) C[(int64_t)row * ldc + col] = alpha * v;
-    });
-  } else {
-    for_each_acc<R, T>(acc, row0, col0, [&](int row, int col, R v) {
-      if (!EDGE || (row < M && col < N)) {
-        R* c = C + (int64_t)row * ldc + col;
-        *c = alpha * v + beta * (*c);
-      }
-    });
-  }
-}
 
 template <typename R, bool A_KMAJOR, bool B_KMAJOR, bool EDGE, int T, int NS = 2>
 __global__ __launch_bounds__(GEMM_THREADS, (T == 128 || NS > 2 ? 2 : 4)) void gemm_mfma_kernel(GemmArgsT<R> p,
diff --git a/gaussian_processes_amd/csrc/gemm_core.h b/gaussian_processes_amd/csrc/gemm_core.h
--- a/gaussian_processes_amd/csrc/gemm_core.h
+++ b/gaussian_processes_amd/csrc/gemm_core.h
@@ -367,6 +367,133 @@
   return {kbeg, kend};
 }
 
+struct TileAt {
+  int x, y, z;
+  static __device__ __forceinline__ TileAt here() { return {(int)blockIdx.x, (int)blockIdx.y, (int)blockIdx.z}; }
+};
+
+template <typename R, bool A_KMAJOR, bool B_KMAJOR, bool EDGE, int T, int NS>
+__device__ __forceinline__ bool gemm_tile_compute(const GemmArgsT<R>& p, int tiles_n, int ntiles, R* smem,
+                                                  typename Real<R>::acc_t (&acc)[T / 32][T / 32], int& ti, int& tj,
+                                                  int& row0, int& col0, R*& C, TileAt at) {
+  constexpr int KT = Real<R>::KT;
+
+  int slab = 0, slab_tiles = 0;
+  const bool slabbed = (T == SLAB_TILE) && p.k_slabs > 0;
+  if (slabbed) {
+    const SlabPlan sp = slab_plan(p.M, p.k_slabs);
+    slab_item(sp, at.x / tiles_n, ti, slab);
+    tj = at.x % tiles_n;
+    slab_tiles = sp.ks;
+  } else if (p.sched != nullptr) {
+    const int e = p.sched[at.x];
+    if (e < 0) return false;
+    ti = e >> 16;
+    tj = e & 0xffff;
+  } else {
+    gemm_walk_tile(at.x, p.reverse, p.out_lower != 0, TILE / T, tiles_n, ntiles, ti, tj);
+  }
+  row0 = ti * T;
+  col0 = tj * T;
+  const int b = at.y, z = at.z;
+  const R* A;
+  const R* B;
+  if (p.nptr > 0) {
+    A = p.Ap[b];
+    B = p.Bp[b];
+    C = p.Cp[b];
+  } else {
+    A = p.A + (int64_t)b * p.sA;
+    B = p.B + (int64_t)b * p.sB;
+    C = p.C + (int64_t)b * p.sC;
+  }
+
+  const KRange kr = gemm_tile_k_range(p.a_tri, p.b_tri, p.K, row0, col0, T);
+  int kbeg = kr.beg, kend = kr.end;
+  if (slabbed) {
+    kbeg = max(kbeg, slab * slab_tiles * T);
+    kend = min(kend, (slab + 1) * slab_tiles * T);
+    C += (int64_t)slab * p.sC;
+  } else if (p.split_k > 1) {
+    const int steps = max(0, kend - kbeg) / KT;
+    const int per = (steps + p.split_k - 1) / p.split_k;
+    const int s0 = min(steps, z * per), s1 = min(steps, (z + 1) * per);
+    kend = kbeg + s1 * KT;
+    kbeg = kbeg + s0 * KT;
+    C += (int64_t)z * p.sC;
+  }
+
+#pragma unroll
+  for (int i = 0; i < T / 32; ++i)
+#pragma unroll
+    for (int j = 0; j < T / 32; ++j) acc[i][j] = acc_zero<R>();
+
+  gemm_mainloop<R, A_KMAJOR, B_KMAJOR, EDGE, T, 0, NS>(A, p.lda, B, p.ldb, p.M, p.N, row0, col0, kbeg, kend, smem, acc,
+                                                       (p.reverse & 4) != 0);
+  return true;
+}
+
+template <typename R, bool A_KMAJOR, bool B_KMAJOR, bool EDGE, int T, int NS, int EPI = 0>
+__device__ __forceinline__ void gemm_tile_body(const GemmArgsT<R>& p, int tiles_n, int ntiles, R* smem, TileAt at = TileAt::here()) {
+  typename Real<R>::acc_t acc[T / 32][T / 32];
+  int ti, tj, row0, col0;
+  R* C;
+  if (!gemm_tile_compute<R, A_KMAJOR, B_KMAJOR, EDGE, T, NS>(p, tiles_n, ntiles, smem, acc, ti, tj, row0, col0, C, at)) return;
+
+  const R alpha = (R)p.alpha, beta = (p.split_k > 1 || (T == SLAB_TILE && p.k_slabs > 0)) ? (R)0 : (R)p.beta;
+  const int64_t ldc = p.ldc;
+  const int M = p.M, N = p.N;
+  if constexpr (EPI != 0) {
+    constexpr int epi = EPI;
+    R* __restrict__ D = p.nptr > 0 ? p.auxp[at.y] : p.aux;
+    double* __restrict__ sumsq = p.nptr > 0 ? p.sumsqp[at.y] : p.sumsq;
+    double ss = 0.0;
+    for_each_acc<R, T>(acc, row0, col0, [&](int row, int col, R v) {
+      if (EDGE && !(row < M && col < N)) return;
+      R o = alpha * v;
+      R* c = C + (int64_t)row * ldc + col;
+      if (epi & 4) {
+        R* dd = D + (int64_t)row * ldc + col;
+        const R d0 = *dd;
+        o += d0;
+        *dd = o + d0;
+      } else if (beta != (R)0) {
+        o += beta * (*c);
+      }
+      if (epi & 1) {
+        if (row >= col) *c = o;
+        if (row > col) C[(int64_t)col * ldc + row] = o;
+      } else {
+        *c = o;
+      }
+      if (epi & 2) ss += (double)o * (double)o;
+    });
+    if (epi & 2) {
+#pragma unroll
+      for (int o = 32; o > 0; o >>= 1) ss += __shfl_down(ss, o);
+      double* red = reinterpret_cast<double*>(smem);
+      __syncthreads();
+      if ((threadIdx.x & 63) == 0) red[threadIdx.x >> 6] = ss;
+      __syncthreads();
+      if (threadIdx.x == 0)
+        sumsq[p.out_lower ? (int64_t)ti * (ti + 1) / 2 + tj : (int64_t)ti * tiles_n + tj] = (red[0] + red[1]) + (red[2] + red[3]);
+    }
+    return;
+  }
+  if (beta == (R)0) {
+    for_each_acc<R, T>(acc, row0, col0, [&](int row, int col, R v) {
+      if (!EDGE || (row < M && col < N)) C[(int64_t)row * ldc + col] = alpha * v;
+    });
+  } else {
+    for_each_acc<R, T>(acc, row0, col0, [&](int row, int col, R v) {
+      if (!EDGE || (row < M && col < N)) {
+        R* c = C + (int64_t)row * ldc + col;
+        *c = alpha * v + beta * (*c);
+      }
+    });
+  }
+}
+
 constexpr int SK_SLOTS = 512;
 struct SkTile {
   int row0, col0, kbeg, ksteps;
diff --git a/gaussian_processes_amd/csrc/kernels.h b/gaussian_processes_amd/csrc/kernels.h
--- a/gaussian_processes_amd/csrc/kernels.h
+++ b/gaussian_processes_amd/csrc/kernels.h
@@ -41,6 +41,21 @@
   int n;
 };
 template <typename R> int launch_chol_leaf_batch(const LeafBatchT<R>& bt, hipStream_t s);
+
+enum LeafAfter { LEAF_TRSM = 1, LEAF_MERGE = 2 };
+template <typename R>
+struct LeafFusedT {
+  LeafBatchT<R> leaf;
+  GemmArgsT<R> prod;
+  uint32_t need;
+  int replicas;
+};
+template <typename R> int launch_chol_leaf_fused(const LeafFusedT<R>& ft, hipStream_t s);
+inline int leaf_replicas(int nb, int cus) {
+  for (int g = 8; g >= 2; g /= 2)
+    if (nb > 0 && (long)nb * g <= (long)cus) return g;
+  return 0;
+}
 
 template <typename R>
 int launch_localker(const Theta& th, const int* pix, int d, int dp, int n_rows, int n_cols, R* C, int64_t ldc,
diff --git a/include/gpfit_mi355x.h b/include/gpfit_mi355x.h
--- a/include/gpfit_mi355x.h
+++ b/include/gpfit_mi355x.h
@@ -196,6 +196,7 @@
                          gpfit_dev_gemm_route_t* out);
 int64_t gpfit_dev_gemm_plan(int is_f32, const gpfit_dev_gemm_args* args, int kind, int32_t* out, int64_t cap);
 int gpfit_dev_gemm(void* stream, int is_f32, const gpfit_dev_gemm_args* args, const gpfit_dev_gemm_args* pair_args);
+int gpfit_dev_leaf_replicas(int nb, int cus);
 int gpfit_dev_ctx_copy(gpfit_ctx* ctx, const char* name, int64_t offset, void* dev, int64_t bytes, int to_ctx);
 int gpfit_dev_ctx_fill(gpfit_ctx* ctx, const char* name, int byte);
 
```

New measurement: 36.66 fits/s (median of 2 runs). No clear change (+0.0%).
